# dnbaker/dashing2

Measured on AMD Instinct MI355X. Metric: all-pairs sketch comparison throughput (pairs/s), higher is better.
Workload: dtype u64

## Files before the change

### dashing2_amd/capi.py

```python
import ctypes as C
import os
import subprocess

import numpy as np

_HERE = os.path.dirname(os.path.abspath(__file__))
LIB_PATH = os.environ.get("D2G_LIB") or os.path.join(_HERE, "libd2g.so")
_lib = None

SIMILARITY, CONTAINMENT, SYMMETRIC_CONTAINMENT, POISSON_LLR, INTERSECTION, UNION_SIZE = range(6)
CMP_AUTO, CMP_DIRECT, CMP_BITSLICE, CMP_PLANES = 0, 1, 2, 3
BITSLICE_OPS_PER_GROUP_EXTRA = 1


TIME_K1, TIME_K2, TIME_K2PREP, TIME_K3, TIME_K0 = 2, 4, 8, 16, 32
TIME_KNN = 64
TIME_DEDUP = 128
TIME_FILTER = 256
TIME_KSET = 512
TIME_SCREEN = 1024


class D2GError(RuntimeError):
    def __init__(self, status, detail=""):
# ... 142 lines not shown
    "d2g_cmp_set_update_dev": (_int, [_vp, _vp, _vp, _vp]),
    "d2g_cmp_set_planes": (_int, [_vp, _vp, _vp, C.POINTER(C.c_uint), C.POINTER(_int), C.POINTER(_f32)]),
    "d2g_cmp_set_status": (_int, [_vp, _vp, _vp]),
    "d2g_cmp_set_sparse_info": (_int, [_vp, _vp, _vp, _vp]),
    "d2g_cmp_set_debug_pairs": (_int, [_vp, _vp, _vp, _vp, _sz, C.POINTER(_sz), _vp]),
    "d2g_cmp_set_sparse_detail": (_int, [_vp, _vp, _vp, _vp]),
    "d2g_sparse_bin_geometry": (_int, [_sz, C.POINTER(C.c_uint32), C.POINTER(C.c_uint32), C.POINTER(C.c_uint32), C.POINTER(_int)]),
    "d2g_warmup": (_int, [_vp, _int]),
    "d2g_device_name": (_int, [_int, C.c_char_p, _sz]),
    "d2g_comm_unique_id": (_int, [_vp]),
    "d2g_comm_create": (_int, [_vp, _vp, _int, _int, C.POINTER(_vp)]),
    "d2g_comm_create_all": (_int, [C.POINTER(_vp), _int, C.POINTER(_vp)]),
    "d2g_comm_destroy": (None, [_vp]),
    "d2g_comm_rank": (_int, [_vp]),
    "d2g_comm_world": (_int, [_vp]),
    "d2g_comm_is_rccl": (_int, [_vp]),
    "d2g_bcast_sigs": (_int, [C.POINTER(_vp), C.POINTER(_vp), _int, _vp, _sz, _sz, C.POINTER(_vp)]),
    "d2g_allpairs_create": (_int, [_vp, _vp, _sz, _sz, C.POINTER(_vp)]),
    "d2g_allpairs_destroy": (None, [_vp]),
    "d2g_allpairs_rows_held": (_int, [_vp, C.POINTER(_sz), C.POINTER(_sz)]),
    "d2g_allpairs_rows_computed": (_int, [_vp, C.POINTER(_sz), C.POINTER(_sz)]),
    "d2g_allpairs_prepare_dev": (_int, [_vp, _vp, _vp]),
    "d2g_allpairs_prepare_all": (_int, [C.POINTER(_vp), _int, C.POINTER(_vp), C.POINTER(_vp)]),
    "d2g_allpairs_operand": (_vp, [_vp]),
    "d2g_allpairs_status": (_int, [_vp, _vp]),
    "d2g_allpairs_chunks": (_int, [_vp]),
    "d2g_allpairs_set_phase_timing": (_int, [_vp, _int]),
    "d2g_allpairs_phase_times": (_int, [_vp, _int, C.POINTER(_int), _vp, _vp, _vp, _vp]),
    "d2g_allpairs_sparse_info": (_int, [_vp, _vp]),
    "d2g_allpairs_step_lut_dev": (_int, [_vp, _vp, _vp, _vp, _vp]),
    "d2g_allpairs_step_eqcount_dev": (_int, [_vp, _vp, _vp, _vp]),
    "d2g_allpairs_step_all": (_int, [C.POINTER(_vp), _int, C.POINTER(_vp), C.POINTER(_vp), C.POINTER(_vp), C.POINTER(_vp)]),
    "d2g_allpairs_enqueue_lut_dev": (_int, [_vp, _vp, _vp, _vp, _vp, _int]),
    "d2g_operand_layout": (_int, [_sz, _sz, C.POINTER(_sz), C.POINTER(_sz)]),
    "d2g_cmp_set_export_operand_dev": (_int, [_vp, _vp, _vp, _vp, _vp]),
    "d2g_cmp_set_from_planes_dev": (_int, [_vp, _sz, _sz, _vp, _vp, C.POINTER(_vp)]),
    "d2g_pack_column_slices_dev": (_int, [_vp, _vp, _sz, _sz, _int, _vp, _vp]),
    "d2g_cmp_set_destroy": (None, [_vp]),
    "d2g_cmp_set_algo": (_int, [_vp]),
    "d2g_cmp_eqcount_ut_dev": (_int, [_vp, _vp, _sz, _sz, _vp, _vp]),
    "d2g_cmp_lut_ut_dev": (_int, [_vp, _vp, _sz, _sz, _vp, _vp, _vp]),
    "d2g_cmp_ut_prefill_dev": (_int, [_vp, _vp, _sz, _sz, _vp, _vp, _vp, _vp]),
    "d2g_cmp_ut_announce_dev": (_int, [_vp, _vp, _sz, _sz, _vp, _vp, _vp]),
    "d2g_cmp_set_forget": (_int, [_vp, _vp]),
    "d2g_cmp_gtlt_ut_dev": (_int, [_vp, _vp, _sz, _sz, _vp, _vp, _vp]),
    "d2g_cmp_eqcount_rect_dev": (_int, [_vp, _vp, _sz, _sz, _sz, _sz, _vp, _vp]),
    "d2g_cmp_gtlt_rect_dev": (_int, [_vp, _vp, _sz, _sz, _sz, _sz, _vp, _vp, _vp]),
    "d2g_cmp_eqcount_ut": (_int, [_vp, _vp, _sz, _sz, _sz, _sz, _int, _vp]),
    "d2g_cmp_dist_ut": (_int, [_vp, _vp, _vp, _sz, _sz, _sz, _sz, _int, _int, _int, _int, _int, _vp]),
    "d2g_ut_partition": (_int, [_sz, _int, C.POINTER(_sz)]),
    "d2g_cmp_set_create_codes_dev": (_int, [_vp, _vp, _sz, _sz, _int, _vp, C.POINTER(_vp)]),
    "d2g_cmp_set_create_codes": (_int, [_vp, _vp, _sz, _sz, _int, C.POINTER(_vp)]),
    "d2g_cmp_set_operand_bytes": (_sz, [_vp]),
    "d2g_cmp_dist_trunc_ut": (_int, [_vp, _vp, _vp, _sz, _sz, _sz, _sz, _int, _int, _int, _int, _int, _vp]),
    "d2g_cmp_knn_dev": (_int, [_vp, _vp, _sz, _sz, _sz, C.c_uint32, _vp, _sz, _vp, _vp, _vp, _sz, _vp]),
    "d2g_knn_finish": (_int, [_vp, _vp, _vp, _sz, _sz, _vp, _sz, _int, _vp, _vp, _vp, _sz, C.POINTER(_sz), C.POINTER(_sz)]),
    "d2g_cmp_set_knn": (_int, [_vp, _vp, _sz, _sz, _vp, _int, _sz, _dbl, _sz, _sz, _vp, _vp, _vp, _sz, C.POINTER(_sz)]),
    "d2g_cmp_knn": (_int, [_vp, _vp, _sz, _sz, _sz, _sz, _int, _int, _int, _int, _sz, _dbl, _sz, _sz, _vp, _vp, _vp, _sz, C.POINTER(_sz)]),
    "d2g_cmp_dedup_dev": (_int, [_vp, _vp, C.c_uint32, _vp, _vp, _sz, _vp]),
    "d2g_dedup_clusters": (_int, [_vp, _sz, _vp, _vp, C.POINTER(_sz)]),
    "d2g_cmp_set_dedup": (_int, [_vp, _vp, _vp, _dbl, _sz, _vp]),
    "d2g_cmp_dedup": (_int, [_vp, _vp, _sz, _sz, _int, _int, _int, _int, _dbl, _sz, _vp]),
}


def sparse_info_dict(a):
    return {"sorted_operand": bool(a[0]), "tiles_listed": int(a[1]), "dense_decided_by_prepare": bool(a[2] & 1), "dense_kernel_ran": bool(a[2] & 2),
            "tiles_and_pair_list": bool(a[2] & 4), "callers_order_kept": bool(a[2] & 8), "ordering_skipped": bool(a[2] & 16), "pairs_listed": int(a[3])}


def lib():
    global _lib
    if _lib is None:
        if os.environ.get("D2G_NO_TORCH_PRELOAD") != "1":
            try:
                import torch
            except Exception:
                pass
        if not os.path.exists(LIB_PATH):
            raise OSError(f"{LIB_PATH} is missing: run `python -c 'import __graft_entry__ as g; g.build()'` "
                          "(dashing2_amd has no CPU fallback)")
        l = C.CDLL(LIB_PATH)
        for name, (res, args) in SIGNATURES.items():
            f = getattr(l, name)
            f.restype = res
            f.argtypes = args
        _lib = l
    return _lib


def _np_ptr(a):
    return a.ctypes.data if a is not None else None


class _Runs:

    def __init__(self, src, canon):
        if hasattr(src, "arrays"):
            src = tuple(src.arrays()) + (src.k,)
        elif src[0] is None:
            src = (None,) + tuple(src[1][:3]) + (src[2],)
        packed, rs, rl, go, self.k = src
        self.packed = None if packed is None else np.ascontiguousarray(packed, np.uint8)
        self.rs, self.rl, self.go = np.ascontiguousarray(rs, np.uint64), np.ascontiguousarray(rl, np.uint32), np.ascontiguousarray(go, np.uint64)
        self.n = self.go.size - 1
        self.args = (_np_ptr(self.packed), 0 if packed is None else self.packed.size, _np_ptr(self.rs), _np_ptr(self.rl), self.rs.size,
                     _np_ptr(self.go), self.n, self.k, int(canon))

    @property
    def nkmers(self):
        return int(self.rl.astype(np.int64).sum()) - (self.k - 1) * self.rl.size if self.rl.size else 0


def wang_hash(x):
    return int(lib().d2g_wang_hash(x & 0xFFFFFFFFFFFFFFFF))


def wang_hash_inverse(x):
    return int(lib().d2g_wang_hash_inverse(x & 0xFFFFFFFFFFFFFFFF))


SCREEN_MAX_KEYS = 1 << 30


def run_emissions(length, k, w=0):
    return int(lib().d2g_run_emissions(int(length), int(k), int(w)))


def screen_table_slots(ndistinct):
    s = _u64()
    rc = lib().d2g_screen_table_slots(ndistinct, C.byref(s))
    if rc:
        raise D2GError(rc)
    return int(s.value)


def epilogue_contain(matches, matchsums, S):
# ... 887 lines not shown
        return int(lib().d2g_kset_slice_bits(self._h))

    def isz_ut_dev(self, r0, r1, out_dev_ptr, stream=None):
        self.ctx._check(lib().d2g_kset_isz_ut_dev(self.ctx._h, self._h, r0, r1, out_dev_ptr, stream))

    def isz_rect_dev(self, a0, a1, b0, b1, out_dev_ptr, stream=None):
        self.ctx._check(lib().d2g_kset_isz_rect_dev(self.ctx._h, self._h, a0, a1, b0, b1, out_dev_ptr, stream))

    def close(self):
        if getattr(self, "_h", None):
            lib().d2g_kset_destroy(self._h)
            self._h = None

    __del__ = close


class OphPlan:
    def __init__(self, ctx, h, n):
        self.ctx, self._h, self.n = ctx, h, n

    def set_filter(self, filt):
        self.ctx._check(lib().d2g_oph_plan_set_filter(self._h, filt._h if filt is not None else None))
        self._filter = filt

    @property
    def nkmers(self):
        return int(lib().d2g_oph_plan_nkmers(self._h))

    @property
    def nbases(self):
        return int(lib().d2g_oph_plan_nbases(self._h))

    def close(self):
        if self._h:
            lib().d2g_oph_plan_destroy(self._h)
            self._h = None

    __del__ = close


class CmpSet:

    def __init__(self, ctx, h, N, S, owned=True):
        self.ctx, self._h, self.N, self.S, self._owned = ctx, h, N, S, owned

    @property
    def algo(self):
        return int(lib().d2g_cmp_set_algo(self._h))

    @property
    def operand_bytes(self):
        return int(lib().d2g_cmp_set_operand_bytes(self._h))

    def close(self):
        if getattr(self, "_h", None):
            if self._owned:
                lib().d2g_cmp_set_destroy(self._h)
            self._h = None

    __del__ = close

    def export_operand_dev(self, planes_out_ptr, meta_out_ptr, stream=None):
        self.ctx._check(lib().d2g_cmp_set_export_operand_dev(self.ctx._h, self._h, planes_out_ptr, meta_out_ptr, stream))

    def update_dev(self, dev_ptr, stream=None):
        self.ctx._check(lib().d2g_cmp_set_update_dev(self.ctx._h, self._h, dev_ptr, stream))

    def status(self, stream=None):
        self.ctx._check(lib().d2g_cmp_set_status(self.ctx._h, self._h, stream))

    def sparse_info(self, stream=None):
        a = np.zeros(4, np.uint32)
        self.ctx._check(lib().d2g_cmp_set_sparse_info(self.ctx._h, self._h, stream, a.ctypes.data))
        return sparse_info_dict(a)

    def sparse_detail(self, stream=None):
        a = np.zeros(10, np.uint64)
        self.ctx._check(lib().d2g_cmp_set_sparse_detail(self.ctx._h, self._h, stream, a.ctypes.data))
        return {"looked": bool(a[0]), "looked_dense": bool(a[1]), "entries": int(a[2]), "family_pairs": int(a[3]), "shared_values": int(a[4]),
                "planes": int(a[5]), "binned": bool(a[6]), "bin_cshift": int(a[7]), "schedule": "merged" if a[8] else "classic", "prepare_kernels": int(a[9])}

    def debug_pairs(self, cap=1 << 24, stream=None):
        buf = np.empty(cap, np.uint64)
        roots = np.empty(self.N, np.uint32)
        n = _sz()
        self.ctx._check(lib().d2g_cmp_set_debug_pairs(self.ctx._h, self._h, stream, buf.ctypes.data, cap, C.byref(n), roots.ctypes.data))
        e = buf[:n.value]
        e = e[e != np.uint64(0xFFFFFFFFFFFFFFFF)]
        return np.stack([(e & np.uint64(0xFFFFFFFF)).astype(np.uint32), (e >> np.uint64(32)).astype(np.uint32)], axis=1), roots

    def planes(self, stream=None):
        md, nb, mean = C.c_uint(), _int(), _f32()
        self.ctx._check(lib().d2g_cmp_set_planes(self.ctx._h, self._h, stream, C.byref(md), C.byref(nb), C.byref(mean)))
        return int(md.value), int(nb.value), float(mean.value)

    def eqcount_ut_dev(self, out_dev_ptr, r0=0, r1=None, stream=None):
        r1 = self.N if r1 is None else r1
        self.ctx._check(lib().d2g_cmp_eqcount_ut_dev(self.ctx._h, self._h, r0, r1, out_dev_ptr, stream))

    def lut_ut_dev(self, lut_dev_ptr, out_dev_ptr, r0=0, r1=None, stream=None):
        r1 = self.N if r1 is None else r1
        self.ctx._check(lib().d2g_cmp_lut_ut_dev(self.ctx._h, self._h, r0, r1, lut_dev_ptr, out_dev_ptr, stream))

    def prefill_ut_dev(self, out_dev_ptr, r0=0, r1=None, lut_dev_ptr=None, stream=None):
        r1 = self.N if r1 is None else r1
        if lut_dev_ptr is None:
# ... 252 lines not shown
```

### dashing2_amd/csrc/d2g_internal.h

```cpp
#pragma once
#include "../../include/d2g.h"
#include <hip/hip_runtime.h>
#include <cstdio>
#include <memory>
#include <string>
#include <utility>

#include <vector>
struct d2g_ctx;
int d2g_hip_status(d2g_ctx *ctx, hipError_t e, const char *what);

template <class T, bool Pinned> class d2g_owned {
    T *p_ = nullptr; size_t cap_ = 0;
public:
    d2g_owned() = default;
    d2g_owned(d2g_owned &&o) noexcept : p_(o.p_), cap_(o.cap_) { o.p_ = nullptr; o.cap_ = 0; }
    d2g_owned &operator=(d2g_owned &&o) noexcept { if (this != &o) { reset(); p_ = o.p_; cap_ = o.cap_; o.p_ = nullptr; o.cap_ = 0; } return *this; }
    ~d2g_owned() { reset(); }
    void reset() { if (p_) (void)(Pinned ? hipHostFree(p_) : hipFree(p_)); p_ = nullptr; cap_ = 0; }
    int alloc(d2g_ctx *ctx, size_t n, const char *what, unsigned flags = hipHostMallocDefault) {
        reset();
        const hipError_t e = Pinned ? hipHostMalloc((void **)&p_, n * sizeof(T), flags) : hipMalloc((void **)&p_, n * sizeof(T));
        if (e != hipSuccess) p_ = nullptr; else cap_ = n;
        return d2g_hip_status(ctx, e, what);
// ... 4 lines not shown
    T *get() const { return p_; }
    operator T *() const { return p_; }
    size_t cap() const { return cap_; }
};
template <class T> using d2g_dev = d2g_owned<T, false>;
template <class T> using d2g_pinned = d2g_owned<T, true>;

template <class H, hipError_t (*Destroy)(H)> class d2g_handle {
protected:
    H h_ = nullptr;
public:
    d2g_handle() = default;
    d2g_handle(d2g_handle &&o) noexcept : h_(o.h_) { o.h_ = nullptr; }
    d2g_handle &operator=(d2g_handle &&o) noexcept { if (this != &o) { reset(); h_ = o.h_; o.h_ = nullptr; } return *this; }
    ~d2g_handle() { reset(); }
    void reset() { if (h_) (void)Destroy(h_); h_ = nullptr; }
    operator H() const { return h_; }
};
struct d2g_stream : d2g_handle<hipStream_t, hipStreamDestroy> {
    hipError_t create(unsigned flags = hipStreamDefault) { reset(); return hipStreamCreateWithFlags(&h_, flags); }
};
struct d2g_event : d2g_handle<hipEvent_t, hipEventDestroy> {
    hipError_t create(unsigned flags = hipEventDefault) { reset(); return hipEventCreateWithFlags(&h_, flags); }
};

struct d2g_evlog {
    std::vector<d2g_event> a, b;
};

struct d2g_tuning {
    std::vector<std::pair<std::string, std::string>> kv;
    const char *get(const char *name) const {
        for (const auto &p : kv) if (p.first == name) return p.second.c_str();
        return nullptr;
    }
};
void d2g_tuning_load(d2g_tuning &t);
struct d2g_k2_tuning {
    bool sparse = true;
    size_t min_n = 8192;
    int link = 1;
    double tile_frac = 0.35;
    int olink = 1;
    int emit_big = 0;
    int ride = 63;
    int merge = 1;
    int remember = 1;
    size_t long_list = 786432;
    int predict = 1;
    int list_form = 0;
    size_t list_div = 8;
    bool sort = true;
    int tagbits_max = 31;
    int nsplit_req = 0;
};
d2g_k2_tuning d2g_k2_tuning_resolve(const d2g_tuning &t);
std::string d2g_k2_tuning_json(const d2g_ctx *ctx);
uint64_t d2g_k2_tuning_hash(const d2g_ctx *ctx);

constexpr int K3_MAXBBITS = 12;
constexpr int K3_ROUND_KEYS = 1400;
constexpr int K3_TARGET = 1024;
constexpr int K3_L1BITS = 8;
constexpr uint64_t K3_SPLIT_MIN = 4 * 1400;
struct d2g_k3_tuning {
    bool compact = false;
    bool light = true;
    uint32_t l1bits = K3_L1BITS;
    uint64_t bucket_keys = K3_TARGET;
    uint64_t sub_keys = K3_TARGET;
    uint64_t split_min = 0;
    size_t subbatch = 0;
    uint32_t round_keys = K3_ROUND_KEYS;
    double guess_scale = 1.0;
    size_t grid_per_cu = 48;
    bool gq_scale_set = false;
    double gq_scale = 2.0;
    uint64_t gq_slack = 256;
    uint64_t sort_keys = K3_TARGET;
};
struct d2g_kset_tuning {
    int split = 0;
    int pbits = -1;
};
d2g_k3_tuning d2g_k3_tuning_resolve(const d2g_tuning &t);
constexpr int MG_MAX_CHUNKS = 4;
void d2g_tuning_resolve(d2g_ctx *ctx);

struct d2g_ctx {
    int device = -1;
    d2g_tuning tune;
    d2g_k2_tuning k2;
    d2g_k3_tuning k3_tune;
    d2g_kset_tuning kset;
    int mgpu_chunks = 0;
    int num_cus = 0;
    std::string last_error;
    int timing = 0;
    d2g_evlog ev_k1, ev_k2, ev_k2prep, ev_k3, ev_k0, ev_knn;
    d2g_evlog ev_k1count;
    d2g_evlog ev_filter;
    d2g_evlog ev_k3s, ev_kset, ev_ksetprep;
    d2g_evlog ev_screen, ev_screenreduce, ev_screenbuild;
    d2g_evlog ev_dedup, ev_dedup_resolve;
    struct d2g_k3_state *k3 = nullptr;
    d2g_dev<uint32_t> knn_band;
// ... 49 lines not shown
```

### dashing2_amd/csrc/d2g_k2.h

```cpp
#pragma once
#include "d2g_internal.h"

#include <algorithm>

struct SpRider { uint32_t *out; size_t cnt; const uint32_t *vsrc; uint32_t vimm, own, piece0; };
constexpr SpRider SP_NO_RIDER{nullptr, 0, nullptr, 0u, 0xFFFFFFFFu, 0u};
constexpr int SP_FILL_PER_THREAD = 8, SP_FILL_THREADS = 256;
inline size_t sp_fill_pieces(size_t cnt) { return div_up<size_t>(cnt / 4 + 1, (size_t)SP_FILL_THREADS * SP_FILL_PER_THREAD); }
#ifndef D2G_SP_RW_M_LINK0
#define D2G_SP_RW_M_LINK0 8
#endif
#ifndef D2G_SP_RW_M_PLANES
#define D2G_SP_RW_M_PLANES 5
#endif
constexpr unsigned SP_RW_PLAN = 6, SP_RW_FLATTEN = 5, SP_RW_COUNT = 5, SP_RW_ATTACH = 5, SP_RW_SCAN = 8, SP_RW_ALL = 35;
constexpr unsigned SP_RW_M_LINK0 = D2G_SP_RW_M_LINK0, SP_RW_M_PLANES = D2G_SP_RW_M_PLANES;

struct SpInit {
    uint32_t *label = nullptr, *ones = nullptr, *zero = nullptr;
    uint32_t n = 0, owords = 0, zwords = 0;
};
#ifdef __HIPCC__
__device__ __forceinline__ void sp_init_part(const SpInit &si, size_t lin, size_t nthreads) {
    if (!si.label) return;
// ... 65 lines not shown
    size_t owner_stride = 0;
    d2g_dev<uint32_t> d_segend;
    d2g_dev<uint32_t> d_posseg;
    d2g_dev<uint32_t> d_hint;
    d2g_dev<uint32_t> d_spz;
    size_t spz_words = 0;
    uint32_t *d_lcnt = nullptr;
    uint32_t *d_gbm = nullptr;
    uint32_t *d_order = nullptr;
    uint32_t *d_plctl = nullptr;
    d2g_dev<uint32_t> d_rowpos;
    d2g_dev<uint32_t> d_rowk;
    d2g_dev<uint32_t> d_rowstream;
    d2g_dev<uint32_t> d_tiles, d_spctl; uint32_t *d_tilebm = nullptr;
    d2g_dev<uint32_t> d_tiles_full; uint32_t *d_fullctl = nullptr;
    bool full_list_valid = false;
    d2g_pinned<uint32_t> h_gaveup; uint32_t *d_gaveup = nullptr;
    d2g_stream fill_stream; d2g_event fill_fork, fill_join;
    d2g_stream samp_stream; d2g_event samp_event;
    d2g_dev<uint32_t> d_samp;
    SpDecision dec;
    SpAnnounced announced;
    SpFilled filled;
    const uint32_t *last_ctl = nullptr;
    d2g_dev<unsigned long long> d_plist;
    size_t plist_cap = 0;
    d2g_dev<unsigned long long> d_plist2;
    uint32_t *d_binc = nullptr;
    d2g_dev<uint32_t> d_bstart;
    d2g_dev<uint32_t> d_cw_ents; d2g_dev<unsigned long long> d_cw_vals; size_t cw_ecap = 0, cw_vcap = 0;
    d2g_dev<uint32_t> d_hoff;
    uint32_t nbins = 0, bin_nch = 0, bin_cshift = 10, bin_nwg = 1;
    bool bin_ok = true;
    size_t tilebm_words = 0, tiles_cap = 0;
};

struct d2g_cmp_set {
    d2g_ctx *ctx = nullptr;
    size_t N = 0, S = 0;
    size_t Npad = 0;
    int algo = D2G_CMP_DIRECT;
    d2g_dev<uint64_t> d_rows;
    d2g_dev<uint64_t> d_cols;
    d2g_dev<uint32_t> d_cplanes;
    int cplanes = 0;
    d2g_dev<uint32_t> own_planes, own_meta;
    uint32_t *d_planes = nullptr;
    d2g_dev<uint32_t> d_stream;
    size_t Nstride = 0;
    int nbits_cap = 0;
    int ntb = 0;
    uint32_t *d_meta = nullptr;
    d2g_dev<uint32_t> d_ids;
    uint32_t T = 0; int logT = 0;
    bool borrowed = false;
    bool want_exchange = false;
    d2g_dev<uint32_t> d_colcnt;
    d2g_dev<uint32_t> d_perm;
    int nsplit = 1;
    bool export_only = false;
    uint32_t *ex_planes = nullptr, *ex_meta = nullptr, *ex_status = nullptr;
    bool managed = false;
    const uint32_t *status_words = nullptr; int n_status = 0;
    std::unique_ptr<SpState> sp;
    bool sparse_ok() const { return sp != nullptr; }
    size_t ncols = 0;
    bool srt_valid = false;
    mutable bool nat_valid = false;
};
constexpr int BS_CC_STRIDE = 8;

struct PairShape;
int  finish_shape(d2g_ctx *ctx, PairShape &sh, unsigned rb);

int  d2g_planes_gtlt(d2g_ctx *ctx, const d2g_cmp_set *set, const PairShape &sh, uint32_t *gt, uint32_t *lt, hipStream_t s);
int  d2g_planes_eq(d2g_ctx *ctx, const d2g_cmp_set *set, const PairShape &sh, uint32_t *eq, hipStream_t s);

void d2g_bitslice_geometry(d2g_cmp_set *set);
int  d2g_bitslice_alloc(d2g_ctx *ctx, d2g_cmp_set *set);
int  d2g_bitslice_prepare(d2g_ctx *ctx, d2g_cmp_set *set, hipStream_t s);
int  d2g_bitslice_export(d2g_ctx *ctx, d2g_cmp_set *set, hipStream_t s);
int  d2g_bitslice_alloc_stream(d2g_ctx *ctx, d2g_cmp_set *set);
int  d2g_bitslice_ensure_natural(d2g_ctx *ctx, const d2g_cmp_set *set, hipStream_t s);
int  d2g_bitslice_managed_sparse_alloc(d2g_ctx *ctx, d2g_cmp_set *set);
int  d2g_bitslice_managed_ready(d2g_ctx *ctx, d2g_cmp_set *set, hipStream_t s);
int  d2g_bitslice_sparse_info(d2g_ctx *ctx, const d2g_cmp_set *set, hipStream_t s, uint32_t *out4);
int  d2g_bitslice_sparse_detail(d2g_ctx *ctx, const d2g_cmp_set *set, hipStream_t s, uint64_t *out10);
SpInit d2g_bitslice_sp_init(const d2g_cmp_set *set);
int  d2g_bitslice_debug_read(d2g_ctx *ctx, const d2g_cmp_set *set, hipStream_t s, uint64_t *pairs_out, size_t cap, size_t *npairs, uint32_t *root_out);
int  d2g_bitslice_status(d2g_ctx *ctx, const d2g_cmp_set *set, hipStream_t s);
int  d2g_bitslice_exporter_create(d2g_ctx *ctx, size_t N, size_t S_local, d2g_cmp_set **out);
void d2g_bitslice_set_export_target(d2g_cmp_set *set, uint32_t *planes, uint32_t *meta, uint32_t *status);
int  d2g_bitslice_prepare_slice(d2g_ctx *ctx, d2g_cmp_set *set, const uint64_t *rows_dev, hipStream_t s);
int  d2g_bitslice_derive_groups(d2g_ctx *ctx, const d2g_cmp_set *set, int g0, int g1, hipStream_t s);
int  d2g_bitslice_ut(d2g_ctx *ctx, const d2g_cmp_set *set, size_t r0, size_t r1, uint32_t *eq_out,
                     const float *lut, float *fout, hipStream_t s);
int  d2g_bitslice_prefill(d2g_ctx *ctx, d2g_cmp_set *set, size_t r0, size_t r1, uint32_t *eq_out, const float *lut, float *fout, hipStream_t s);
int  d2g_bitslice_announce(d2g_ctx *ctx, d2g_cmp_set *set, size_t r0, size_t r1, uint32_t *eq_out, const float *lut, float *fout);
void d2g_bitslice_forget(d2g_cmp_set *set);
int  d2g_bitslice_rect(d2g_ctx *ctx, const d2g_cmp_set *set, size_t a0, size_t a1, size_t b0, size_t b1,
                       uint32_t *eq_out, hipStream_t s);
```

### dashing2_amd/csrc/d2g_k2.hip

```cpp
#include "d2g_internal.h"
#include "d2g_k2.h"
#include "d2g_k2_shape.h"
#include <algorithm>
#include <new>
#include <vector>

namespace {

constexpr int K2_THREADS = 256;
constexpr int K2_IW = 8;
constexpr int K2_JR = 4;
constexpr int K2_RB = 4 * K2_IW;
constexpr int K2_CB = 64 * K2_JR;
constexpr int K2_TC = 2;

}
int finish_shape(d2g_ctx *ctx, PairShape &sh, unsigned rb) {
    sh.rb = rb;
    sh.nrt = (unsigned)div_up<size_t>(sh.i_hi - sh.i_lo, rb);
    sh.ct0 = (unsigned)(sh.j_lo / 256);
    sh.nct = (unsigned)(div_up<size_t>(sh.j_hi, 256) - sh.ct0);
    size_t total = 0;
    for (unsigned c = 0; c < sh.nct; ++c) total += tiles_in_column(sh, c);
    D2G_CHECK(ctx, total < (1ull << 31), "pair tile grid too large; shard rows");
// ... 98 lines not shown
    } else {
        uint32_t val[K2_IW][K2_JR];
#pragma unroll
        for (int i = 0; i < K2_IW; ++i)
#pragma unroll
            for (int c = 0; c < K2_JR; ++c) val[i][c] = store.value(acc[i][c]);
#pragma unroll
        for (int i = 0; i < K2_IW; ++i) {
            const size_t ii = iw0 + i;
            if (ii >= sh.i_hi) break;
#pragma unroll
            for (int c = 0; c < K2_JR; ++c) {
                const size_t jj = j0 + lane + 64 * c;
                if (jj < sh.j_hi && jj >= sh.j_lo && (!sh.ut || jj > ii)) store.put(out_pos(sh, ii, jj), val[i][c]);
            }
        }
    }
}

template <bool GTLT, class Store>
int launch_direct(d2g_ctx *ctx, const d2g_cmp_set *set, PairShape sh, Store store, hipStream_t s) {
    if (int rc = finish_shape(ctx, sh, K2_RB)) return rc;
    if (sh.nvalid_total == 0) return D2G_OK;
    d2g_timer tm(ctx, &ctx->ev_k2, s);
    hipLaunchKernelGGL((k2_direct_kernel<GTLT, Store>), dim3(sh.per_xcd * 8), dim3(K2_THREADS), 0, s,
                       set->d_rows, set->d_cols, set->S, set->Npad, sh, store);
    tm.stop();
    D2G_HIP(ctx, hipGetLastError());
    return D2G_OK;
}

}

namespace {
__global__ __launch_bounds__(256) void k2_pack_slices_kernel(const uint64_t *__restrict__ rows, size_t n, size_t S, size_t Sl,
                                                             uint64_t *__restrict__ out) {
    const size_t i = (size_t)blockIdx.x * 256 + threadIdx.x;
    if (i >= n * S) return;
    const size_t r = i / S, c = i - r * S, q = c / Sl;
    out[(q * n + r) * Sl + (c - q * Sl)] = rows[i];
}
}


extern "C" {

void d2g_cmp_set_destroy(d2g_cmp_set *set) {
    if (!set) return;
    (void)hipSetDevice(set->ctx->device);
    delete set;
}

int d2g_cmp_set_algo(const d2g_cmp_set *set) { return set ? set->algo : D2G_ERR_INVALID; }

size_t d2g_cmp_set_operand_bytes(const d2g_cmp_set *set) {
    if (!set) return 0;
    return (set->d_rows.cap() + set->d_cols.cap()) * sizeof(uint64_t) +
           (set->own_planes.cap() + set->d_stream.cap() + (set->sp ? set->sp->d_stream_s.cap() : 0) + set->d_cplanes.cap()) * sizeof(uint32_t);
}

#define D2G_NO_CODE_SET(ctx, set, what) D2G_CHECK(ctx, (set)->algo != D2G_CMP_PLANES, what ": not available for a set of truncated codes")

static int cmp_set_load(d2g_ctx *ctx, d2g_cmp_set *set, const uint64_t *sig_bits_dev, hipStream_t s) {
    const size_t N = set->N, S = set->S;
    if (set->d_rows) D2G_HIP(ctx, hipMemcpyAsync(set->d_rows, sig_bits_dev, N * S * sizeof(uint64_t), hipMemcpyDeviceToDevice, s));
    d2g_timer tm(ctx, &ctx->ev_k2prep, s);
    launch_transpose(ctx, sig_bits_dev, set->d_cols, N, S, set->Npad, set->algo == D2G_CMP_BITSLICE ? set->d_meta + set->ntb : nullptr,
                     set->algo == D2G_CMP_BITSLICE ? d2g_bitslice_sp_init(set) : SpInit{}, s);
    int rc = D2G_OK;
    if (set->algo == D2G_CMP_BITSLICE) rc = d2g_bitslice_prepare(ctx, set, s);
    tm.stop();
    if (rc) return rc;
    D2G_HIP(ctx, hipGetLastError());
    return D2G_OK;
}

}

int d2g_bitslice_prepare_slice(d2g_ctx *ctx, d2g_cmp_set *set, const uint64_t *rows_dev, hipStream_t s) {
    d2g_timer tm(ctx, &ctx->ev_k2prep, s);
    launch_transpose(ctx, rows_dev, set->d_cols, set->N, set->S, set->Npad, set->d_meta + set->ntb, d2g_bitslice_sp_init(set), s);
    const int rc = d2g_bitslice_prepare(ctx, set, s);
    tm.stop();
    if (rc) return rc;
    D2G_HIP(ctx, hipGetLastError());
    return D2G_OK;
}

extern "C" {

int d2g_cmp_set_create_dev(d2g_ctx *ctx, const uint64_t *sig_bits_dev, size_t N, size_t S, int algo,
                           void *stream, d2g_cmp_set **out) {
    if (!ctx || !out) return D2G_ERR_INVALID;
    *out = nullptr;
    D2G_CHECK(ctx, N >= 1 && S >= 1, "cmp_set: empty matrix");
    D2G_CHECK(ctx, S < (1ull << 31), "cmp_set: sketchsize too large");
    D2G_CHECK(ctx, sig_bits_dev != nullptr, "cmp_set: null signatures");
    D2G_CHECK(ctx, algo == D2G_CMP_AUTO || algo == D2G_CMP_DIRECT || algo == D2G_CMP_BITSLICE, "cmp_set: bad algo");
    D2G_HIP(ctx, hipSetDevice(ctx->device));
    hipStream_t s = as_stream(stream);
    d2g_cmp_set *set = new (std::nothrow) d2g_cmp_set();
    if (!set) return D2G_ERR_NOMEM;
    set->ctx = ctx; set->N = N; set->S = S;
    set->Npad = div_up<size_t>(N, K2_CB) * K2_CB;
    if (int rc = set->d_cols.alloc(ctx, set->Npad * S, "cmp_set alloc")) { d2g_cmp_set_destroy(set); return rc; }
    set->algo = D2G_CMP_DIRECT;
// ... 326 lines not shown
```

### dashing2_amd/csrc/d2g_k2_bitslice.hip

```cpp
#include "d2g_internal.h"
#include "d2g_k2.h"
#include "d2g_k2_shape.h"
#include <chrono>
#include <cstring>
#include <algorithm>
#include <vector>

namespace {

typedef uint32_t u32x16 __attribute__((ext_vector_type(16)));
typedef u32x16 __attribute__((aligned(4))) u32x16_u;
constexpr uint32_t BS_EMPTY = 0xFFFFFFFFu;
constexpr int BS_RANK_THREADS = 1024;

constexpr uint32_t BS_DUP = 0x80000000u;
constexpr uint32_t BS_UNIQ = 0x80000000u;
constexpr uint32_t BS_PENDING = 0x40000000u;
constexpr int BS_LOG_TLDS_MAX = 15;

__device__ __forceinline__ uint32_t bs_hash(uint64_t v, int logT) {
    return (uint32_t)((v * 0x9E3779B97F4A7C15ull) >> (64 - logT));
}

constexpr uint32_t BS_SPLIT_SHIFT = 28, BS_RANK_MASK = (1u << BS_SPLIT_SHIFT) - 1u;
#ifdef D2G_RANK_TRACE
__device__ unsigned long long g_rank_trace[8192 * 16];
#define RK_STAMP(k) do { if (threadIdx.x == 0 && blockIdx.x < 8192 && (k) < 16) g_rank_trace[blockIdx.x * 16 + (k)] = __builtin_amdgcn_s_memrealtime(); } while (0)
#else
#define RK_STAMP(k) do { } while (0)
#endif
template <bool MULTI, bool FAST>
__global__ __launch_bounds__(BS_RANK_THREADS) void bs_rank_kernel(const uint64_t *__restrict__ cols, size_t N, size_t Npad,
                                                                  uint32_t T, int logT, uint32_t *ids_all, uint32_t *colcnt,
                                                                  uint32_t *status, int tagbits_max, uint32_t S, int nsplit,
                                                                  uint32_t *__restrict__ owner_all, size_t ostride) {
    extern __shared__ __attribute__((aligned(16))) uint32_t own[];
    const uint32_t split = MULTI ? blockIdx.x / S : 0u;
    const size_t t = MULTI ? blockIdx.x - split * S : blockIdx.x;
    const uint32_t htag = (MULTI && nsplit > 1) ? split << BS_SPLIT_SHIFT : 0u;
    const uint64_t *col = cols + t * Npad;
    uint32_t *ids = ids_all + t * Npad;
    const int tid = threadIdx.x;
    const int logTl = logT < BS_LOG_TLDS_MAX ? logT : BS_LOG_TLDS_MAX;
    const uint32_t Tl = 1u << logTl, mask = Tl - 1, nparts = MULTI ? (T >> logTl) : 1u;
    const uint32_t part_lo = MULTI ? split * (nparts / (uint32_t)nsplit) : 0u, part_hi = MULTI ? part_lo + nparts / (uint32_t)nsplit : 1u;
    __shared__ uint32_t wave_tot[BS_RANK_THREADS / 64];
    __shared__ uint32_t running;
    constexpr uint32_t BS_MAXFIX = 64;
    __shared__ uint32_t nfix, fix_j[BS_MAXFIX], fix_h[BS_MAXFIX];
    RK_STAMP(0);
    if (tid == 0) { running = 1; nfix = 0; }
    const int lane = tid & 63, wave = tid >> 6;
    uint32_t *owner = (owner_all && nsplit == 1) ? owner_all + t * ostride : nullptr;
    const int ib0 = 32 - __clz((uint32_t)N);
    const uint32_t ownmask = (ib0 >= 32 ? 0xFFFFFFFFu : (1u << ib0) - 1u) & ~BS_DUP;

    auto compact = [&]() {
        uint32_t cnt = 0;
        for (uint32_t h = tid; h < Tl; h += BS_RANK_THREADS) {
            const uint32_t cur = own[h];
            cnt += (cur != BS_EMPTY) && (cur & BS_DUP);
        }
        uint32_t incl = cnt;
        for (int o = 1; o < 64; o <<= 1) { const uint32_t x = __shfl_up(incl, o); if (lane >= o) incl += x; }
        if (lane == 63) wave_tot[wave] = incl;
        __syncthreads();
        uint32_t woff = 0, tot = 0;
        for (int w = 0; w < BS_RANK_THREADS / 64; ++w) {
            const uint32_t x = wave_tot[w];
            if (w < wave) woff += x;
            tot += x;
        }
        uint32_t r = running + woff + (incl - cnt);
        for (uint32_t h = tid; h < Tl; h += BS_RANK_THREADS) {
            const uint32_t cur = own[h];
            if (cur != BS_EMPTY) {
                if ((cur & BS_DUP) && owner) owner[r - 1] = cur & ownmask;
                own[h] = (cur & BS_DUP) ? (r++ | htag) : BS_UNIQ;
            }
        }
        __syncthreads();
        if (tid == 0) running += tot;
        __syncthreads();
    };
    const int ib = 32 - __clz((uint32_t)N);
    const uint32_t idxmask = (ib >= 32 ? 0xFFFFFFFFu : (1u << ib) - 1u) & ~BS_DUP;
    const uint32_t tagfield = ~BS_DUP & ~idxmask & (ib + tagbits_max >= 31 ? 0xFFFFFFFFu : (1u << (ib + tagbits_max)) - 1u);
    auto slot_word = [&](uint64_t prod, uint32_t j) {
        return j | ((uint32_t)((prod << logT) >> 33) & tagfield);
    };
    auto insert = [&](uint64_t v, uint32_t j, uint32_t h) {
        const uint32_t mine = slot_word(v * 0x9E3779B97F4A7C15ull, j);
        for (uint32_t probes = 0; probes < Tl; ++probes) {
            const uint32_t cur = atomicCAS(&own[h], BS_EMPTY, mine);
            if (cur == BS_EMPTY) return h;
            if (!((cur ^ mine) & tagfield) && col[cur & idxmask] == v) {
                if (!(cur & BS_DUP)) atomicOr(&own[h], BS_DUP);
                return h;
            }
            h = (h + 1) & mask;
        }
        atomicOr(status, 1u);
        return h;
    };

    constexpr int PF = 12;
    if constexpr (FAST) {
        uint64_t v[PF];
        uint32_t hs[PF];
#pragma unroll
        for (int i = 0; i < PF; ++i) {
            const size_t j = (size_t)i * BS_RANK_THREADS + tid;
            v[i] = j < N ? col[j] : 0;
        }
        for (uint32_t h = tid; h < Tl; h += BS_RANK_THREADS) own[h] = BS_EMPTY;
        __syncthreads();
        RK_STAMP(1);
        uint32_t candidate = 0;
#pragma unroll
        for (int i = 0; i < PF; ++i) {
            const size_t j = (size_t)i * BS_RANK_THREADS + tid;
            hs[i] = 0;
            if (j < N) {
                const uint64_t prod = v[i] * 0x9E3779B97F4A7C15ull;
                const uint32_t mine = slot_word(prod, (uint32_t)j);
                uint32_t h = (uint32_t)(prod >> (64 - logT)) & mask, probes = 0;
                for (; probes < Tl; ++probes) {
                    const uint32_t cur = atomicCAS(&own[h], BS_EMPTY, mine);
                    if (cur == BS_EMPTY) break;
                    if (!((cur ^ mine) & tagfield)) { candidate |= 1u << i; break; }
                    h = (h + 1) & mask;
                }
                if (probes == Tl) atomicOr(status, 1u);
                hs[i] = h;
            }
        }
        constexpr int CB = 2;
        uint32_t redo = 0;
#ifdef D2G_RANK_TRACE
        __syncthreads();
        RK_STAMP(2);
#endif
#pragma unroll
        for (int c = 0; c < PF; c += CB) {
            uint32_t o[CB];
            uint64_t w[CB];
#pragma unroll
            for (int g = 0; g < CB; ++g)
                if (candidate >> (c + g) & 1) o[g] = own[hs[c + g]];
#pragma unroll
            for (int g = 0; g < CB; ++g)
                if (candidate >> (c + g) & 1) w[g] = col[o[g] & idxmask];
#pragma unroll
            for (int g = 0; g < CB; ++g)
                if (candidate >> (c + g) & 1) {
                    if (w[g] == v[c + g]) {
                        if (!(o[g] & BS_DUP)) atomicOr(&own[hs[c + g]], BS_DUP);
                    } else redo |= 1u << (c + g);
                }
            __builtin_amdgcn_sched_barrier(0);
        }
        const uint32_t skip = redo;
        while (redo) {
            const int i = __ffs(redo) - 1;
            redo &= redo - 1;
            const uint32_t j = (uint32_t)i * BS_RANK_THREADS + tid;
            const uint64_t vv = col[j];
            const uint32_t h2 = insert(vv, j, bs_hash(vv, logT) & mask);
            const uint32_t k = atomicAdd(&nfix, 1u);
            if (k < BS_MAXFIX) { fix_j[k] = j; fix_h[k] = h2; }
            else atomicOr(status, 1u);
        }
        __syncthreads();
        RK_STAMP(3);
        compact();
        RK_STAMP(4);
#pragma unroll
        for (int i = 0; i < PF; ++i) {
            const size_t j = (size_t)i * BS_RANK_THREADS + tid;
            if (j < N && !(skip >> i & 1)) ids[j] = own[hs[i]];
        }
#ifdef D2G_RANK_TRACE
        __syncthreads();
        RK_STAMP(5);
#endif
        for (uint32_t k = tid; k < nfix && k < BS_MAXFIX; k += BS_RANK_THREADS) ids[fix_j[k]] = own[fix_h[k]];
        if (tid == 0) { colcnt[t * BS_CC_STRIDE] = running - 1; colcnt[t * BS_CC_STRIDE + 5] = running - 1; }
        return;
    }

    const bool tagged = MULTI && nsplit > 1;
    for (uint32_t part = part_lo; part < part_hi; ++part) {
        const uint32_t ptag = BS_PENDING | (tagged ? part << 15 : 0u);
        for (uint32_t h = tid; h < Tl; h += BS_RANK_THREADS) own[h] = BS_EMPTY;
        __syncthreads();
        constexpr int PG = 8;
        const bool mine_known = N <= (size_t)8 * PG * BS_RANK_THREADS;
        unsigned long long mine_all = 0;
        int batch = 0;
        for (size_t j0 = 0; j0 < N; j0 += (size_t)PG * BS_RANK_THREADS) {
            uint64_t v[PG];
            uint32_t hs[PG];
#pragma unroll
            for (int i = 0; i < PG; ++i) {
                const size_t j = j0 + (size_t)i * BS_RANK_THREADS + tid;
                v[i] = j < N ? col[j] : 0;
            }
            uint32_t mineb = 0, candidate = 0, redo = 0;
#pragma unroll
            for (int i = 0; i < PG; ++i) {
                const size_t j = j0 + (size_t)i * BS_RANK_THREADS + tid;
                const uint64_t prod = v[i] * 0x9E3779B97F4A7C15ull;
                const uint32_t hh = (uint32_t)(prod >> (64 - logT));
                hs[i] = 0;
                if (j < N && (!MULTI || (hh >> logTl) == part)) {
                    mineb |= 1u << i;
                    const uint32_t mine = slot_word(prod, (uint32_t)j);
                    uint32_t h = hh & mask, probes = 0;
                    for (; probes < Tl; ++probes) {
                        const uint32_t cur = atomicCAS(&own[h], BS_EMPTY, mine);
                        if (cur == BS_EMPTY) break;
                        if (!((cur ^ mine) & tagfield)) { candidate |= 1u << i; break; }
                        h = (h + 1) & mask;
                    }
                    if (probes == Tl) atomicOr(status, 1u);
                    hs[i] = h;
                }
            }
            {
                uint32_t o[PG];
                uint64_t w[PG];
#pragma unroll
                for (int i = 0; i < PG; ++i)
                    if (candidate >> i & 1) o[i] = own[hs[i]];
#pragma unroll
                for (int i = 0; i < PG; ++i)
                    if (candidate >> i & 1) w[i] = col[o[i] & idxmask];
#pragma unroll
                for (int i = 0; i < PG; ++i)
                    if (candidate >> i & 1) {
                        if (w[i] == v[i]) { if (!(o[i] & BS_DUP)) atomicOr(&own[hs[i]], BS_DUP); }
                        else redo |= 1u << i;
                    }
            }
#pragma unroll
            for (int i = 0; i < PG; ++i) {
                const size_t j = j0 + (size_t)i * BS_RANK_THREADS + tid;
                if ((mineb & ~redo) >> i & 1) ids[j] = hs[i] | (MULTI ? ptag : 0u);
                else if (MULTI && !tagged && part == 0 && j < N && !(redo >> i & 1)) ids[j] = 0;
            }
            while (redo) {
                const int i = __ffs(redo) - 1;
                redo &= redo - 1;
                const size_t j = j0 + (size_t)i * BS_RANK_THREADS + tid;
                const uint64_t vv = col[j];
                ids[j] = insert(vv, (uint32_t)j, bs_hash(vv, logT) & mask) | (MULTI ? ptag : 0u);
            }
            if (batch < 8) mine_all |= (unsigned long long)mineb << (8 * batch);
            ++batch;
        }
        __syncthreads();
        RK_STAMP(1 + 2 * (part - part_lo));
        compact();
        batch = 0;
        for (size_t j0 = 0; j0 < N; j0 += (size_t)PG * BS_RANK_THREADS, ++batch) {
            uint32_t sl[PG];
            const uint32_t mb = mine_known ? (uint32_t)(mine_all >> (8 * batch)) & 0xFFu : 0xFFu;
#pragma unroll
            for (int i = 0; i < PG; ++i) {
                const size_t j = j0 + (size_t)i * BS_RANK_THREADS + tid;
                sl[i] = (j < N && (mb >> i & 1)) ? ids[j] : 0;
            }
#pragma unroll
            for (int i = 0; i < PG; ++i) {
                const size_t j = j0 + (size_t)i * BS_RANK_THREADS + tid;
                if (j < N && (mb >> i & 1) && (mine_known || !MULTI || (tagged ? (sl[i] & ~0x7FFFu) == ptag : (sl[i] & BS_PENDING) != 0)))
                    ids[j] = own[sl[i] & (tagged ? 0x7FFFu : ~BS_PENDING)];
            }
        }
        __syncthreads();
        RK_STAMP(2 + 2 * (part - part_lo));
    }
    if (tid == 0) { colcnt[t * BS_CC_STRIDE + split] = running - 1; if (nsplit == 1) colcnt[t * BS_CC_STRIDE + 5] = running - 1; }
}

__device__ __forceinline__ int live_planes(const uint32_t *meta, int tb) {
    const uint32_t md = meta[tb];
    return md <= 1 ? 1 : 32 - __clz(md);
}

__device__ __forceinline__ size_t stream_slot(const uint32_t *meta, int tb) {
    size_t q = 0;
    for (int t = 0; t < tb; ++t) q += (size_t)live_planes(meta, t);
    return q;
}

__device__ __forceinline__ size_t stream_slot_wave(const uint32_t *meta, int tb) {
    const int lane = threadIdx.x & 63;
    uint32_t q = 0;
    for (int t0 = 0; t0 < tb; t0 += 64) {
        const int t = t0 + lane;
        uint32_t v = t < tb ? (uint32_t)live_planes(meta, t) : 0u;
        for (int o = 32; o > 0; o >>= 1) v += __shfl_xor(v, o);
        q += v;
    }
    return (size_t)__builtin_amdgcn_readfirstlane(q);
}

__device__ __forceinline__ void sp_ride_piece(const SpRider &r, size_t piece) {
    typedef uint32_t u32x4 __attribute__((ext_vector_type(4)));
    const uint32_t v = r.vsrc ? r.vsrc[0] : r.vimm;
    const size_t head = min(r.cnt, (size_t)((16 - ((uintptr_t)r.out & 15)) & 15) / 4);
    u32x4 *body = reinterpret_cast<u32x4 *>(r.out + head);
    const size_t nb = (r.cnt - head) / 4;
    const size_t end = min((piece + 1) * (size_t)2048, nb);
    for (size_t i = piece * 2048 + threadIdx.x; i < end; i += blockDim.x) __builtin_nontemporal_store(u32x4{v, v, v, v}, &body[i]);
    if (piece == 0) {
        if (threadIdx.x < head) r.out[threadIdx.x] = v;
        const size_t tail0 = head + nb * 4;
        if (tail0 + threadIdx.x < r.cnt) r.out[tail0 + threadIdx.x] = v;
    }
}
__device__ __forceinline__ void sp_ride(const SpRider &r) { sp_ride_piece(r, (size_t)r.piece0 + (blockIdx.x - r.own)); }
#define SP_RIDE_OR_WORK(r) do { if (blockIdx.x >= (r).own) { sp_ride(r); return; } } while (0)
__global__ __launch_bounds__(256) void sp_side_fill_kernel(SpRider r, uint32_t pieces) {
    for (size_t p = blockIdx.x; p < pieces; p += gridDim.x) sp_ride_piece(r, p);
}
constexpr uint32_t SP_SIDE_FILL_PIECES = 32768;
inline unsigned sp_side_fill_grid(const d2g_ctx *ctx, uint32_t pieces, size_t words, size_t N, size_t S) {
    const double need = (double)words * 4.0 / (1.3 * 21.0 * (double)N * ((double)S / 1024.0));
// ... 65 lines not shown
            if (t < Spad) d2s[t] = d2;
            unsigned long long todo = __ballot(t < Spad);
            while (todo) {
                const int k = __shfl(cls, __ffsll((long long)todo) - 1);
                const unsigned long long m = __ballot(cls == k && t < Spad);
                const uint32_t ci = (uint32_t)(31 - k) * nchunk + t / 64;
                if (cls == k && t < Spad) mine[it] = ci << 6 | (uint32_t)__popcll(m & ((1ull << lane) - 1));
                if (lane == 0) cell[(uint32_t)(31 - k) * nchunk + (t - lane) / 64] = __popcll(m);
                todo &= ~m;
            }
        }
    }
    __syncthreads();
    {
        constexpr int CPT = 32 * (BS_PLAN_MAXS / 64) / T;
        const uint32_t c0 = (uint32_t)CPT * tid;
        uint32_t v[CPT], sum = 0;
#pragma unroll
        for (int x = 0; x < CPT; ++x) { v[x] = c0 + x < ncell ? cell[c0 + x] : 0u; sum += v[x]; }
        uint32_t incl = sum;
        for (int o = 1; o < 64; o <<= 1) { const uint32_t x = __shfl_up(incl, o); if (lane >= o) incl += x; }
        if (lane == 63) wave_tot[wave] = incl;
        __syncthreads();
        uint32_t ex = incl - sum;
        for (int w = 0; w < wave; ++w) ex += wave_tot[w];
#pragma unroll
        for (int x = 0; x < CPT; ++x) { if (c0 + x < ncell) cell[c0 + x] = ex; ex += v[x]; }
    }
    __syncthreads();
#pragma unroll
    for (int it = 0; it < IT; ++it) {
        const uint32_t t = (uint32_t)it * T + tid;
        if (t < Spad) perm_s[cell[mine[it] >> 6] + (mine[it] & 63u)] = (uint16_t)t;
    }
    __syncthreads();
    for (uint32_t p = tid; p < Spad; p += T) { const uint32_t t = perm_s[p]; perm[p] = t < S ? t : BS_NOCOL; }
    for (int g = tid; g < ntb; g += T) {
        uint32_t mx = 0;
        for (uint32_t x = 0; x < 32; ++x) mx = max(mx, d2s[perm_s[(uint32_t)g * 32 + x]]);
        meta[g] = mx + 1;
        if (ex_meta) ex_meta[g] = mx + 1;
    }
}

__global__ __launch_bounds__(BS_PLAN_THREADS) void bs_colplan_kernel(BsPlanArgs pa, SpRider rider) {
    SP_RIDE_OR_WORK(rider);
    extern __shared__ __attribute__((aligned(16))) uint32_t plan_lds[];
    bs_colplan_body<BS_PLAN_THREADS>(pa, bs_plan_lds(plan_lds, (uint32_t)pa.ntb * 32u));
}

constexpr int BS_FORM_STREAM = 1, BS_FORM_EXCHANGE = 2;
constexpr size_t BS_SLACK = 64;
struct BsPlanesArgs {
    const uint32_t *ids; size_t N, Npad; uint32_t *planes, *stream; size_t Nstride; int nbits_cap; const uint32_t *meta; int forms;
    const uint32_t *perm, *colcnt, *sperm;
};
BsPlanesArgs planes_args_of(const d2g_cmp_set *set, uint32_t *planes, int forms) {
    return BsPlanesArgs{set->d_ids, set->N, set->Npad, planes, set->d_stream, set->Nstride, set->nbits_cap, set->d_meta, forms, set->d_perm, set->d_colcnt, nullptr};
}
template <bool SPLIT>
__device__ __forceinline__ void bs_planes_body(const BsPlanesArgs &a, size_t bx, size_t tb) {
    const uint32_t *__restrict__ ids = a.ids, *__restrict__ meta = a.meta, *__restrict__ perm = a.perm, *__restrict__ colcnt = a.colcnt, *__restrict__ sperm = a.sperm;
    uint32_t *__restrict__ planes = a.planes, *__restrict__ stream = a.stream;
    const size_t N = a.N, Npad = a.Npad, Nstride = a.Nstride;
    const int nbits_cap = a.nbits_cap, forms = a.forms;
    const size_t jpos = bx * 256 + threadIdx.x;
    const size_t slot = (forms & BS_FORM_STREAM) ? stream_slot_wave(meta, (int)tb) : 0;
    if (jpos >= Nstride) return;
    const size_t j = sperm ? (size_t)sperm[jpos] : jpos;
    const int nbits = live_planes(meta, (int)tb);
    typedef const u32x16_u __attribute__((address_space(4))) *slots_ptr;
    const u32x16_u pa = *(slots_ptr)(uintptr_t)(perm + tb * 32), pb = *(slots_ptr)(uintptr_t)(perm + tb * 32 + 16);
    uint32_t id[32];
#pragma unroll
    for (int x = 0; x < 32; ++x) {
        const uint32_t t = x < 16 ? pa[x] : pb[x - 16];
        const bool real = t != BS_NOCOL && j < N;
        uint32_t w = real ? ids[(size_t)t * Npad + j] : 0u;
        if (SPLIT && real && !(w >> 31)) w = (w & BS_RANK_MASK) + colcnt[(size_t)t * BS_CC_STRIDE + (w >> BS_SPLIT_SHIFT)];
        id[x] = w;
    }
    uint32_t u = 0;
#pragma unroll
    for (int x = 0; x < 32; ++x) u |= (id[x] >> 31) << x;
    uint32_t *dst = planes + tb * (size_t)(nbits_cap + 1) * Nstride + jpos;
    const bool ex = forms & BS_FORM_EXCHANGE, st = forms & BS_FORM_STREAM;
    uint32_t *sdst = st ? stream + slot * 2 * Nstride + jpos : nullptr;
    for (int b = 0; b < nbits; ++b) {
        uint32_t w = 0;
#pragma unroll
        for (int x = 0; x < 32; ++x) w |= ((id[x] >> b) & 1u) << x;
        if (ex) dst[(size_t)b * Nstride] = w;
        if (st) {
            sdst[(size_t)(2 * b) * Nstride] = w;
            sdst[(size_t)(2 * b + 1) * Nstride] = w | u;
        }
    }
    if (ex) {
        uint32_t uw = u;
        if (jpos >= Npad && jpos < Npad + 32) { const uint32_t t = perm[tb * 32 + (jpos - Npad)]; uw = t != BS_NOCOL ? colcnt[(size_t)t * BS_CC_STRIDE + 4] : 0u; }
        dst[(size_t)nbits_cap * Nstride] = uw;
    }
}
template <bool SPLIT>
__global__ __launch_bounds__(256) void bs_planes_kernel(BsPlanesArgs a) { bs_planes_body<SPLIT>(a, blockIdx.x, blockIdx.y); }

__global__ __launch_bounds__(256) void bs_derive_kernel(const uint32_t *__restrict__ planes, uint32_t *__restrict__ stream,
                                                        size_t Nstride, int nbits_cap, const uint32_t *__restrict__ meta, int tb0) {
    const size_t j = (size_t)blockIdx.x * 256 + threadIdx.x;
    const size_t tb = (size_t)tb0 + blockIdx.y;
    if (j >= Nstride) return;
    const int nbits = live_planes(meta, (int)tb);
    const uint32_t *src = planes + tb * (size_t)(nbits_cap + 1) * Nstride + j;
    uint32_t *sdst = stream + stream_slot(meta, (int)tb) * 2 * Nstride + j;
    const uint32_t u = j + BS_SLACK < Nstride ? src[(size_t)nbits_cap * Nstride] : 0u;
    for (int b = 0; b < nbits; ++b) {
        const uint32_t w = src[(size_t)b * Nstride];
        sdst[(size_t)(2 * b) * Nstride] = w;
        sdst[(size_t)(2 * b + 1) * Nstride] = w | u;
    }
}

constexpr int BS_THREADS = 256;
constexpr int BS_CB = 256;

constexpr unsigned BITOP3_C_OR_A_XOR_B = 0xAA | (0xF0 ^ 0xCC);

#ifndef D2G_BS_WPE
#define D2G_BS_WPE 7
#endif
#ifndef D2G_BS_JR
#define D2G_BS_JR 2
#endif
constexpr int BS_IW = 16;
constexpr int BS_JR = D2G_BS_JR;

__device__ __forceinline__ bool sp_dense_mode(const uint32_t *__restrict__ ctl, uint32_t cand);
#include "d2g_k2_patch.h"


template <int JR>
struct BsOperands {
    u32x16_u sa;
    uint32_t vb[JR];
};

template <int JR>
__device__ __forceinline__ BsOperands<JR> bs_fetch(const uint32_t *&ptr, uint32_t coff, size_t step) {
    __builtin_amdgcn_s_waitcnt(0xc07f);
    __builtin_amdgcn_sched_barrier(0);
    BsOperands<JR> o;
    typedef const u32x16_u __attribute__((address_space(4))) *row_words_ptr;
    o.sa = *(row_words_ptr)(uintptr_t)ptr;
    uint32_t co = coff;
    asm volatile("" : "+v"(co));
#pragma unroll
    for (int c = 0; c < JR; ++c)
        o.vb[c] = *reinterpret_cast<const uint32_t *>(reinterpret_cast<const char *>(ptr) + co + 256 * c);
// ... 114 lines not shown

#include "d2g_k2_sparse.h"

int refresh_borrowed(d2g_ctx *ctx, const d2g_cmp_set *set, hipStream_t s) {
    if (!set->borrowed || set->managed) return D2G_OK;
    return d2g_bitslice_derive_groups(ctx, set, 0, set->ntb, s);
}


template <class Store>
int launch_bitslice(d2g_ctx *ctx, const d2g_cmp_set *set, PairShape sh, Store store, hipStream_t s) {
    if (int rc = finish_shape(ctx, sh, BS_JR == 2 ? 32u : 64u)) return rc;
    if (sh.nvalid_total == 0) return D2G_OK;
    if (int rc = refresh_borrowed(ctx, set, s)) return rc;
    if (int rc = d2g_bitslice_ensure_natural(ctx, set, s)) return rc;
    d2g_timer tm(ctx, &ctx->ev_k2, s);
    hipLaunchKernelGGL((k2_bitslice_kernel<BS_JR, Store>), dim3(sh.per_xcd * 8), dim3(BS_THREADS), 0, s, set->d_stream,
                       set->Nstride, set->d_meta, set->ntb, (uint32_t)set->S, sh, store, (const uint32_t *)nullptr, 0u, SpPatchArgs{});
    tm.stop();
    D2G_HIP(ctx, hipGetLastError());
    return D2G_OK;
}

}

void d2g_bitslice_geometry(d2g_cmp_set *set) {
    set->nbits_cap = 1;
    while ((1ull << set->nbits_cap) < set->N / 2 + 2) ++set->nbits_cap;
    set->ntb = (int)div_up<size_t>(set->S, 32);
    set->Nstride = set->Npad + BS_SLACK;
}

int d2g_bitslice_alloc_stream(d2g_ctx *ctx, d2g_cmp_set *set) {
    return set->d_stream.alloc(ctx, ((size_t)set->ntb * set->nbits_cap + 1) * 2 * set->Nstride, "bitslice alloc");
}

namespace {
int alloc_prepare_workspace(d2g_ctx *ctx, d2g_cmp_set *set) {
    const size_t N = set->N, S = set->S, Npad = set->Npad;
    if (N >= (1ull << 30)) { ctx->last_error = "bitslice: N too large"; return D2G_ERR_UNSUPPORTED; }
    d2g_bitslice_geometry(set);
    set->T = 64; set->logT = 6;
    while ((uint64_t)set->T * 2 < (uint64_t)N * 3) { set->T <<= 1; ++set->logT; }
    set->nsplit = 1;
    if (set->logT > BS_LOG_TLDS_MAX && N < (1ull << BS_SPLIT_SHIFT)) {
        const uint32_t nparts = set->T >> BS_LOG_TLDS_MAX;
        int want = 1;
        while (want < 4 && (uint32_t)want * 2 <= nparts && S * (size_t)want < (size_t)std::max(ctx->num_cus, 1)) want *= 2;
        if (ctx->k2.nsplit_req && (uint32_t)ctx->k2.nsplit_req <= nparts) want = ctx->k2.nsplit_req;
        set->nsplit = want;
    }
    const char *what = "bitslice alloc";
    int rc;
    if ((rc = set->d_ids.alloc(ctx, S * Npad, what)) ||
        (rc = d2g_hip_status(ctx, hipMemset(set->d_ids, 0, S * Npad * sizeof(uint32_t)), what)) ||
        (rc = set->d_colcnt.alloc(ctx, S * BS_CC_STRIDE, what)) ||
        (rc = set->d_perm.alloc(ctx, (size_t)set->ntb * 32, what)) ||
        (rc = set->own_meta.alloc(ctx, (size_t)(set->ntb + 4), what)) ||
        (rc = d2g_hip_status(ctx, hipMemset(set->own_meta, 0, (size_t)(set->ntb + 4) * sizeof(uint32_t)), what))) return rc;
    set->d_meta = set->own_meta;
    return D2G_OK;
}
int launch_planes(d2g_ctx *ctx, const d2g_cmp_set *set, uint32_t *planes, int forms, hipStream_t s) {
    const dim3 grid((unsigned)div_up<size_t>(set->Nstride, 256), (unsigned)set->ntb);
    const bool split = set->logT > BS_LOG_TLDS_MAX && set->nsplit > 1;
    hipLaunchKernelGGL(split ? bs_planes_kernel<true> : bs_planes_kernel<false>, grid, dim3(256), 0, s, planes_args_of(set, planes, forms));
    D2G_HIP(ctx, hipGetLastError());
    return D2G_OK;
}
struct JoinOnExit {
    hipStream_t s; hipEvent_t ev = nullptr;
    ~JoinOnExit() { if (ev) (void)hipStreamWaitEvent(s, ev, 0); }
};
}

int d2g_bitslice_alloc(d2g_ctx *ctx, d2g_cmp_set *set) {
    if (int rc = alloc_prepare_workspace(ctx, set)) return rc;
    if (int rc = set->own_planes.alloc(ctx, (size_t)set->ntb * (set->nbits_cap + 1) * set->Nstride, "bitslice alloc")) return rc;
    set->d_planes = set->own_planes;
    if (int rc = d2g_bitslice_alloc_stream(ctx, set)) return rc;
    set->ncols = set->S;
    if (sparse_enabled(ctx, set->N) && set->S < 65536 && sp_alloc(ctx, set) != D2G_OK) (void)hipGetLastError();
    if (set->sparse_ok() && set->nsplit == 1) {
        set->sp->owner_stride = set->N / 2 + 8;
        if (set->sp->d_owner.alloc(ctx, set->S * set->sp->owner_stride, "bitslice owner alloc") != D2G_OK) (void)hipGetLastError();
    }
    return D2G_OK;
}

int d2g_bitslice_prepare(d2g_ctx *ctx, d2g_cmp_set *set, hipStream_t s) {
    const size_t N = set->N, S = set->S, Npad = set->Npad;
    SpState *const sp = set->sp.get();
    const bool sparse_path = sp && !set->export_only && !set->want_exchange;
    JoinOnExit join{s};
    if (sp) {
        sp->dec.skip_cached = sparse_path ? (sp_will_skip(ctx, *sp) ? 1 : 0) : -1;
        sp->announced.begin(ctx->k2.ride, sparse_path && sp->dec.skip_cached != 1);
    }
    if (sp && sp->announced.riding() >= SP_SIDE_FILL_PIECES) {
        if (!sp->fill_stream) {
            if (sp->fill_stream.create(hipStreamNonBlocking) != hipSuccess || sp->fill_fork.create(hipEventDisableTiming) != hipSuccess ||
                sp->fill_join.create(hipEventDisableTiming) != hipSuccess) { (void)hipGetLastError(); sp->fill_stream.reset(); sp->fill_fork.reset(); sp->fill_join.reset(); }
        }
        if (sp->fill_stream) {
            hipStream_t fs = sp->fill_stream;
            D2G_HIP(ctx, hipEventRecord(sp->fill_fork, s));
            D2G_HIP(ctx, hipStreamWaitEvent(fs, sp->fill_fork, 0));
            join.ev = sp->fill_join;
            const uint32_t pieces = sp->announced.riding();
            const SpRider all = sp->announced.take_all();
            const unsigned fgrid = sp_side_fill_grid(ctx, pieces, all.cnt, N, S);
            hipLaunchKernelGGL(sp_side_fill_kernel, dim3(fgrid), dim3(256), 0, fs, all, pieces);
            D2G_HIP(ctx, hipEventRecord(sp->fill_join, fs));
        }
    }
    const bool multi = set->logT > BS_LOG_TLDS_MAX;
    const int nsplit = multi ? set->nsplit : 1;
    {
        const int logTl = set->logT < BS_LOG_TLDS_MAX ? set->logT : BS_LOG_TLDS_MAX;
        const size_t lds = (size_t(1) << logTl) * sizeof(uint32_t);
        void (*kern)(const uint64_t *, size_t, size_t, uint32_t, int, uint32_t *, uint32_t *, uint32_t *, int, uint32_t, int, uint32_t *, size_t) = bs_rank_kernel<false, false>;
        if (multi) kern = bs_rank_kernel<true, false>;
        else if (N <= (size_t)12 * BS_RANK_THREADS) kern = bs_rank_kernel<false, true>;
        if (lds > 48 * 1024)
            D2G_HIP(ctx, hipFuncSetAttribute((const void *)kern, hipFuncAttributeMaxDynamicSharedMemorySize, (int)lds));
        if (nsplit > 1) D2G_HIP(ctx, hipMemsetAsync(set->d_ids, 0, S * Npad * sizeof(uint32_t), s));
        hipLaunchKernelGGL(kern, dim3((unsigned)(S * nsplit)), dim3(BS_RANK_THREADS), lds, s, set->d_cols, N, Npad, set->T, set->logT,
                           set->d_ids, set->d_colcnt, set->d_meta + set->ntb, ctx->k2.tagbits_max, (uint32_t)S, nsplit,
                           (sp && nsplit == 1) ? sp->d_owner.get() : (uint32_t *)nullptr, sp ? sp->owner_stride : 0);
        if (sp) sp->dec.kernels = 2 + (join.ev ? 1 : 0);
        const bool look = sparse_path && sp_sample_due(ctx, set);
        if (look) { if (int rc = sp_sample_enqueue(ctx, set, s)) return rc; if (sp->dec.sample_pending) sp->dec.kernels += 2; }
        const bool merged = sparse_path && !look && ctx->k2.merge && nsplit == 1 && sp->d_owner && ctx->k2.olink && ctx->k2.link && sp->dec.skip_cached != 1;
        if (sp) sp->dec.merged = merged;
        if (!merged) {
            unsigned g = 1; const SpRider rd = sp ? sp->announced.take(1, SP_RW_PLAN, false, 1, &g) : SP_NO_RIDER;
            const BsPlanArgs pa{set->d_colcnt, (uint32_t)S, set->ntb, nsplit, set->d_perm, set->d_meta, set->d_meta + set->ntb, set->ex_meta, set->ex_status, ctx->k2.sort ? 1 : 0};
            hipLaunchKernelGGL(bs_colplan_kernel, dim3(g), dim3(BS_PLAN_THREADS), bs_plan_lds_words((uint32_t)set->ntb * 32u, pa.sort) * 4, s, pa, rd);
            if (sp) sp->dec.kernels += 1;
        }
    }
    if (sparse_path) {
        if (!sp->dec.merged) { if (int rc = launch_planes(ctx, set, set->d_planes, BS_FORM_STREAM, s)) return rc; sp->dec.kernels += 1; }
        if (int rc = sp_sample_collect(ctx, set, s)) return rc;
        if (int rc = sp_prepare_order(ctx, set, nsplit > 1, s)) return rc;
        if (int rc = sp_permute(ctx, set, s)) return rc;
        set->srt_valid = true; set->nat_valid = true;
        if (sp->announced.riding()) sp->filled.set_by_riders(sp->announced);
        else sp->filled.void_after_prepare();
        sp->announced.served();
        D2G_HIP(ctx, hipGetLastError());
        return D2G_OK;
    }
    if (sp) sp->announced.served();
    const int forms = set->export_only ? BS_FORM_EXCHANGE : (BS_FORM_STREAM | (set->want_exchange ? BS_FORM_EXCHANGE : 0));
    if (int rc = launch_planes(ctx, set, set->export_only ? set->ex_planes : set->d_planes, forms, s)) return rc;
    if (sp) sp->dec.kernels += 1;
    set->srt_valid = false; set->nat_valid = true;
    return D2G_OK;
}

SpInit d2g_bitslice_sp_init(const d2g_cmp_set *set) { return sp_init_of(set); }

int d2g_bitslice_ensure_natural(d2g_ctx *ctx, const d2g_cmp_set *set, hipStream_t s) {
    if (set->nat_valid || set->borrowed || set->export_only) return D2G_OK;
    if (int rc = launch_planes(ctx, set, set->d_planes, BS_FORM_STREAM, s)) return rc;
    set->nat_valid = true;
    return D2G_OK;
}

int d2g_bitslice_export(d2g_ctx *ctx, d2g_cmp_set *set, hipStream_t s) {
    if (set->borrowed || set->want_exchange || set->export_only) return D2G_OK;
    set->want_exchange = true;
    return launch_planes(ctx, set, set->d_planes, BS_FORM_EXCHANGE, s);
}

int d2g_bitslice_exporter_create(d2g_ctx *ctx, size_t N, size_t S_local, d2g_cmp_set **out) {
    *out = nullptr;
    d2g_cmp_set *set = new (std::nothrow) d2g_cmp_set();
    if (!set) return D2G_ERR_NOMEM;
    set->ctx = ctx; set->N = N; set->S = S_local;
// ... 120 lines not shown
    return D2G_OK;
}

int d2g_bitslice_sparse_detail(d2g_ctx *ctx, const d2g_cmp_set *set, hipStream_t s, uint64_t *out8) {
    uint32_t binned = 0;
    if (set->sp) D2G_HIP(ctx, hipMemcpyAsync(&binned, set->sp->d_plctl + SP_PL_BINNED, 4, hipMemcpyDeviceToHost, s));
    D2G_HIP(ctx, hipStreamSynchronize(s));
    if (!set->sp) return D2G_OK;
    const SpState &sp = *set->sp;
    out8[0] = sp.dec.looked ? 1 : 0; out8[1] = sp.dec.looked_dense ? 1 : 0;
    if (sp.dec.looked) for (int x = 0; x < 4; ++x) out8[2 + x] = sp.dec.samp_sums[x];
    out8[6] = binned ? 1 : 0; out8[7] = sp.bin_cshift;
    out8[8] = sp.dec.merged ? 1 : 0; out8[9] = sp.dec.kernels;
    return D2G_OK;
}

int d2g_sparse_bin_geometry(size_t N, uint32_t *cshift, uint32_t *nch, uint32_t *nbins, int *binned_ok) {
    if (!N) return D2G_ERR_INVALID;
    const SpBinGeom g = sp_bin_geometry(N);
    if (cshift) *cshift = g.cshift;
    if (nch) *nch = g.nch;
    if (nbins) *nbins = g.nbins;
    if (binned_ok) *binned_ok = g.ok ? 1 : 0;
    return D2G_OK;
}

int d2g_bitslice_debug_read(d2g_ctx *ctx, const d2g_cmp_set *set, hipStream_t s, uint64_t *pairs_out, size_t cap, size_t *npairs, uint32_t *root_out ) {
    *npairs = 0;
    if (!set->srt_valid || !set->sp) { D2G_HIP(ctx, hipStreamSynchronize(s)); return D2G_OK; }
    const SpState &sp = *set->sp;
    uint32_t n = 0;
    D2G_HIP(ctx, hipMemcpyAsync(&n, sp.d_plctl, 4, hipMemcpyDeviceToHost, s));
    D2G_HIP(ctx, hipStreamSynchronize(s));
    const size_t m = std::min<size_t>(std::min<size_t>(n, sp.plist_cap), cap);
    if (m && pairs_out) D2G_HIP(ctx, hipMemcpy(pairs_out, sp.d_plist, m * 8, hipMemcpyDeviceToHost));
    if (root_out) D2G_HIP(ctx, hipMemcpy(root_out, sp.d_label + set->Npad, set->N * 4, hipMemcpyDeviceToHost));
    *npairs = m;
    return D2G_OK;
}

uint64_t d2g_k2_tuning_hash(const d2g_ctx *ctx) {
    const d2g_k2_tuning &t = ctx->k2;
    const long long v[] = {t.sparse, (long long)t.min_n, t.link, (long long)(t.tile_frac * 1e6), t.olink, t.emit_big, t.ride, t.remember, (long long)t.list_div, (long long)t.long_list,
                           t.list_form, t.predict, t.sort ? 1 : 0, t.tagbits_max, t.nsplit_req, t.merge};
    uint64_t h = 1469598103934665603ull;
    for (long long x : v) for (int b = 0; b < 8; ++b) { h ^= (uint64_t)(x >> (8 * b)) & 0xFF; h *= 1099511628211ull; }
    return h;
}

std::string d2g_k2_tuning_json(const d2g_ctx *ctx) {
    const d2g_k2_tuning &t = ctx->k2;
    char b[640];
    std::snprintf(b, sizeof b, "{\"D2G_BS_SPARSE\": %d, \"D2G_BS_SPARSE_MIN_N\": %zu, \"D2G_BS_SORT\": %d, \"D2G_SP_LINK\": %d, \"D2G_SP_OLINK\": %d, \"D2G_SP_TILE_FRAC\": %.3f, "
                  "\"D2G_SP_LIST_DIV\": %zu, \"D2G_SP_LONG_LIST\": %zu, \"D2G_SP_LIST_FORM\": %d, \"D2G_SP_PREDICT\": %d, \"D2G_SP_REMEMBER\": %d, \"D2G_SP_RIDE\": %d, \"D2G_SP_EMIT_BIG\": %d, \"D2G_K2_MERGE\": %d}",
                  t.sparse ? 1 : 0, t.min_n, t.sort ? 1 : 0, t.link, t.olink, t.tile_frac, t.list_div, t.long_list, t.list_form, t.predict, t.remember, t.ride, t.emit_big, t.merge);
    return b;
}

void d2g_warm_k2_bitslice() { hipFuncAttributes a; (void)hipFuncGetAttributes(&a, reinterpret_cast<const void *>(&bs_colplan_kernel)); }

#ifdef D2G_RANK_TRACE
extern "C" int d2g_debug_rank_trace(unsigned long long *out, size_t n) {
    return hipMemcpyFromSymbol(out, HIP_SYMBOL(g_rank_trace), std::min<size_t>(n, 8192 * 16) * 8) == hipSuccess ? 0 : -1;
}
#endif
#ifdef D2G_SP_TRACE
extern "C" int d2g_debug_emit_trace(unsigned long long *out, size_t n) {
    return hipMemcpyFromSymbol(out, HIP_SYMBOL(g_emit_trace), std::min<size_t>(n, 4096 * 16) * 8) == hipSuccess ? 0 : -1;
}
extern "C" int d2g_debug_sp_trace(unsigned long long *out, size_t n) {
    return hipMemcpyFromSymbol(out, HIP_SYMBOL(g_sp_trace), std::min<size_t>(n, 16384 * 8) * 8) == hipSuccess ? 0 : -1;
}
#endif
```

### dashing2_amd/csrc/d2g_k2_sparse.h

```cpp
constexpr uint32_t SP_NONE = 0xFFFFFFFFu;
constexpr uint32_t SP_SAMPLE_ROWS = 16, SP_SAMPLE_FAM = 4, SP_SAMPLE_COLS = 32;
constexpr unsigned long long SP_NULL_ENTRY = ~0ull;
#ifndef D2G_SP_KS
#define D2G_SP_KS 8
#endif
#ifndef D2G_SP_WPE
#define D2G_SP_WPE 8
#endif

__device__ __forceinline__ uint32_t sp_rank(uint32_t w, const uint32_t *__restrict__ colcnt, size_t t, bool split) {
    if ((w >> 31) || w == 0) return 0;
    return split ? (w & BS_RANK_MASK) + colcnt[t * BS_CC_STRIDE + (w >> BS_SPLIT_SHIFT)] : w;
}

__device__ __forceinline__ uint32_t sp_ld(const uint32_t *p) { return __hip_atomic_load(p, __ATOMIC_RELAXED, __HIP_MEMORY_SCOPE_AGENT); }

__device__ __forceinline__ uint32_t sp_find(uint32_t *label, uint32_t l) {
    for (int h = 0; h < 64; ++h) {
        const uint32_t p = sp_ld(&label[l]);
        if (p == l) break;
        const uint32_t g = sp_ld(&label[p]);
        if (g != p) label[l] = g;
        l = p;
    }
    return l;
}
__device__ __forceinline__ bool sp_union(uint32_t *label, uint32_t a, uint32_t b) {
    for (int it = 0; it < 64; ++it) {
        a = sp_find(label, a); b = sp_find(label, b);
        if (a == b) return true;
        if (a < b) { const uint32_t x = a; a = b; b = x; }
        if (atomicCAS(&label[a], a, b) == a) return true;
    }
    return false;
}

constexpr uint32_t SP_UDONE = 0x40000000u, SP_R2MASK = 0x3FFFFFFFu;
template <int MODE>
__global__ __launch_bounds__(1024) void sp_link_kernel(const uint32_t *__restrict__ ids, size_t N, size_t Npad, uint32_t ncols, const uint32_t *__restrict__ colcnt,
                                                       int split, uint32_t cap, uint32_t stride, uint32_t *label, uint32_t *__restrict__ hint) {
    extern __shared__ uint32_t sp_l[];
    const size_t pair = (size_t)blockIdx.x * stride;
    const size_t t1 = 2 * pair, t2 = t1 + 1;
    if (t2 >= ncols) return;
    const uint32_t d2 = colcnt[t1 * BS_CC_STRIDE + 4];
    if (d2 == 0) return;
    const uint32_t nv = min(d2, cap), T = blockDim.x;
    uint32_t *r2 = sp_l, *mn = sp_l + nv, *any = sp_l + 2 * (size_t)nv;
    for (uint32_t r = threadIdx.x; r < (MODE ? 2u : 3u) * nv; r += T) sp_l[r] = SP_NONE;
    __syncthreads();
    constexpr int U = 4;
    for (size_t j0 = 0; j0 < N; j0 += (size_t)T * U) {
        uint32_t w1[U], w2[U], lb[U];
#pragma unroll
        for (int x = 0; x < U; ++x) {
            const size_t j = j0 + (size_t)x * T + threadIdx.x;
            w1[x] = j < N ? ids[t1 * Npad + j] : 0u;
            w2[x] = j < N ? ids[t2 * Npad + j] : 0u;
            lb[x] = j < N ? sp_ld(&label[j]) : SP_NONE;
        }
#pragma unroll
        for (int x = 0; x < U; ++x) {
            const uint32_t j = (uint32_t)(j0 + (size_t)x * T + threadIdx.x);
            const uint32_t a = sp_rank(w1[x], colcnt, t1, split != 0), b = sp_rank(w2[x], colcnt, t2, split != 0);
            if (!a || a > nv) continue;
            if (MODE == 0) any[a - 1] = j;
            if (!b) continue;
            const uint32_t old = atomicCAS(&r2[a - 1], SP_NONE, b);
            if (old == SP_NONE || (old & SP_R2MASK) == b) {
                atomicMin(&mn[a - 1], lb[x]);
            }
        }
    }
    __syncthreads();
    uint32_t *myhint = hint + (size_t)(pair & 1u) * Npad;
    for (size_t j0 = 0; j0 < N; j0 += (size_t)T * U) {
        uint32_t w1[U], w2[U], lb[U];
#pragma unroll
        for (int x = 0; x < U; ++x) {
            const size_t j = j0 + (size_t)x * T + threadIdx.x;
            w1[x] = j < N ? ids[t1 * Npad + j] : 0u;
            w2[x] = j < N ? ids[t2 * Npad + j] : 0u;
            lb[x] = j < N ? sp_ld(&label[j]) : 0u;
        }
#pragma unroll
        for (int x = 0; x < U; ++x) {
            const uint32_t j = (uint32_t)(j0 + (size_t)x * T + threadIdx.x);
            const uint32_t a = sp_rank(w1[x], colcnt, t1, split != 0), b = sp_rank(w2[x], colcnt, t2, split != 0);
            if (!a || a > nv) continue;
            const uint32_t rr = r2[a - 1];
            const bool match = b && rr != SP_NONE && (rr & SP_R2MASK) == b;
            if (MODE == 0) {
                if (match) {
                    const uint32_t m = mn[a - 1];
                    if (m < lb[x]) label[j] = m;
                } else {
                    const uint32_t h = any[a - 1];
                    if (h != j) myhint[j] = h;
                }
            } else if (match) {
                const uint32_t m = mn[a - 1];
                if (m != lb[x] && !(atomicOr(&r2[a - 1], SP_UDONE) & SP_UDONE)) (void)sp_union(label, lb[x], m);
            }
        }
    }
}

constexpr uint32_t SP_OWNER_MASK = 0x7FFFFFFFu;
struct SpOlinkArgs { const uint32_t *ids; size_t N, Npad; uint32_t ncols; uint32_t *owner; size_t ostride; uint32_t stride; uint32_t *label, *hint; };
template <int MODE>
__device__ __forceinline__ void sp_olink_body(const SpOlinkArgs &a, size_t bx, size_t by) {
    const uint32_t *__restrict__ ids = a.ids;
    uint32_t *__restrict__ owner = a.owner, *label = a.label, *__restrict__ hint = a.hint;
    const size_t N = a.N, Npad = a.Npad, ostride = a.ostride;
    const size_t pair = by * a.stride;
    const size_t t1 = 2 * pair, t2 = t1 + 1;
    if (t2 >= a.ncols) return;
    const size_t j0 = (bx * 256 + threadIdx.x) * 4;
    if (j0 >= N) return;
    typedef uint32_t u32x4 __attribute__((ext_vector_type(4)));
    const u32x4 w1 = *reinterpret_cast<const u32x4 *>(ids + t1 * Npad + j0);
    const u32x4 w2 = *reinterpret_cast<const u32x4 *>(ids + t2 * Npad + j0);
    const u32x4 lb = *reinterpret_cast<const u32x4 *>(label + j0);
    uint32_t *myhint = hint + (size_t)(pair & 1u) * Npad;
    uint32_t o[4], r2o[4], lo[4];
#pragma unroll
    for (int x = 0; x < 4; ++x) {
        const uint32_t r1 = w1[x];
        o[x] = (r1 && !(r1 >> 31) && j0 + x < N) ? owner[t1 * ostride + r1 - 1] & SP_OWNER_MASK : SP_NONE;
    }
#pragma unroll
    for (int x = 0; x < 4; ++x) {
        const bool live = o[x] != SP_NONE && o[x] != (uint32_t)(j0 + x);
        r2o[x] = live ? ids[t2 * Npad + o[x]] : 0u;
        lo[x] = live ? label[o[x]] : 0u;
        if (!live) o[x] = SP_NONE;
    }
#pragma unroll
    for (int x = 0; x < 4; ++x) {
        if (o[x] == SP_NONE) continue;
        const uint32_t j = (uint32_t)(j0 + x), r2 = w2[x];
        const bool match = r2 && !(r2 >> 31) && r2 == r2o[x];
        if (MODE == 0) {
            if (match) {
                if (lo[x] < lb[x]) label[j] = lo[x]; else if (lb[x] < lo[x]) label[o[x]] = lb[x];
            } else myhint[j] = o[x];
        } else if (match && lb[x] != lo[x]) {
            uint32_t *ow = &owner[t1 * ostride + w1[x] - 1];
            if (!(atomicOr(ow, ~SP_OWNER_MASK) & ~SP_OWNER_MASK)) (void)sp_union(label, lb[x], lo[x]);
        }
    }
}
template <int MODE>
__global__ __launch_bounds__(256) void sp_olink_kernel(SpOlinkArgs a) { sp_olink_body<MODE>(a, blockIdx.x, blockIdx.y); }

__device__ __forceinline__ void sp_flatten_body(uint32_t *label, size_t N, size_t bx) {
    const size_t j = bx * 256 + threadIdx.x;
    if (j >= N) return;
    uint32_t l = (uint32_t)j;
    for (int h = 0; h < 64; ++h) {
        const uint32_t p = label[l];
        if (p == l) break;
        const uint32_t g = label[p];
        if (g != p) label[l] = g;
        l = p;
    }
    if (label[l] == l) label[j] = l;
}
__global__ __launch_bounds__(256) void sp_flatten_kernel(uint32_t *label, size_t N, SpRider rider) {
    SP_RIDE_OR_WORK(rider);
    sp_flatten_body(label, N, blockIdx.x);
}

__global__ __launch_bounds__(256) void sp_link0_plan_kernel(BsPlanArgs pa, SpOlinkArgs la, uint32_t nx, SpRider rider) {
    SP_RIDE_OR_WORK(rider);
    extern __shared__ __attribute__((aligned(16))) uint32_t plan_lds[];
    if (blockIdx.x == 0) { bs_colplan_body<256>(pa, bs_plan_lds(plan_lds, (uint32_t)pa.ntb * 32u)); return; }
    const uint32_t b = blockIdx.x - 1u;
    sp_olink_body<0>(la, b % nx, b / nx);
}
__global__ __launch_bounds__(256) void bs_planes_flatten_kernel(BsPlanesArgs a, uint32_t gx, uint32_t nflat, uint32_t *label, SpRider rider) {
    SP_RIDE_OR_WORK(rider);
    if (blockIdx.x < nflat) { sp_flatten_body(label, a.N, blockIdx.x); return; }
    const uint32_t b = blockIdx.x - nflat;
    bs_planes_body<false>(a, b % gx, b / gx);
}

__global__ __launch_bounds__(256) void sp_attach_kernel(uint32_t *__restrict__ root, uint32_t *__restrict__ cnt, const uint32_t *__restrict__ hint, size_t N, size_t Npad,
                                                        const uint32_t *__restrict__ order, SpRider rider) {
    SP_RIDE_OR_WORK(rider);
    const size_t j = (size_t)blockIdx.x * 256 + threadIdx.x;
    if (j >= N || order[2]) return;
    if (root[j] != (uint32_t)j || sp_ld(&cnt[j]) != 1u) return;
    const uint32_t a = hint[j], b = hint[Npad + j];
    if (a == SP_NONE && b == SP_NONE) return;
    const uint32_t ra = a != SP_NONE ? sp_ld(&root[a]) : SP_NONE, rb = b != SP_NONE ? sp_ld(&root[b]) : SP_NONE;
    if (ra != SP_NONE && rb != SP_NONE && ra != rb) return;
    const uint32_t r = ra != SP_NONE ? ra : rb;
    if (r == (uint32_t)j || sp_ld(&cnt[r]) < 2u) return;
    root[j] = r;
    atomicAdd(&cnt[r], 1u);
    cnt[j] = 0;
}

template <int NW = 16>
__device__ __forceinline__ uint32_t sp_block_scan(uint32_t v, uint32_t *wave_tot, uint32_t *total) {
    const int lane = threadIdx.x & 63, wave = threadIdx.x >> 6;
    uint32_t incl = v;
    for (int o = 1; o < 64; o <<= 1) { const uint32_t x = __shfl_up(incl, o); if (lane >= o) incl += x; }
    __syncthreads();
    if (lane == 63) wave_tot[wave] = incl;
    __syncthreads();
    uint32_t woff = 0, tot = 0;
    for (int w = 0; w < NW; ++w) { const uint32_t x = wave_tot[w]; if (w < wave) woff += x; tot += x; }
    *total = tot;
    return woff + incl - v;
}

template <int NW>
__device__ __forceinline__ unsigned long long sp_block_scan64(unsigned long long v, unsigned long long *wave_tot, unsigned long long *total) {
    const int lane = threadIdx.x & 63, wave = threadIdx.x >> 6;
    unsigned long long incl = v;
    for (int o = 1; o < 64; o <<= 1) { const unsigned long long x = __shfl_up(incl, o); if (lane >= o) incl += x; }
    __syncthreads();
    if (lane == 63) wave_tot[wave] = incl;
    __syncthreads();
    unsigned long long woff = 0, tot = 0;
    for (int w = 0; w < NW; ++w) { const unsigned long long x = wave_tot[w]; if (w < wave) woff += x; tot += x; }
    *total = tot;
    return woff + incl - v;
}

__device__ __forceinline__ uint32_t sp_seg_est(uint32_t c) {
    c = min(c, 32768u);
    return c >= 32 ? 16u * ((c + 31) / 32 + 1) * ((c + 255) / 256 + 1) : (c >= 2 ? c : 0u);
}

constexpr int SP_MAX_HOPS = 64;
// ... 79 lines not shown
    __syncthreads();
    if (tid == 0) { const uint32_t keep = (s_big || order[2] || s_est > seg_tile_limit + 1024) ? 1u : 0u; order[0] = keep; *gaveup = keep; }
}
__device__ __forceinline__ void sp_segtiles(uint32_t a, uint32_t b, uint32_t CW, uint32_t *__restrict__ gbm) {
    if (b - a < 2) return;
    const uint32_t cb0 = a >> 8, cb1 = (b - 1) >> 8;
    for (uint32_t rb = a >> 5; rb <= (b - 1) >> 5; ++rb)
        for (uint32_t cw = cb0 >> 5; cw <= cb1 >> 5; ++cw) {
            const uint32_t lo = cw == (cb0 >> 5) ? (cb0 & 31) : 0u, hi = cw == (cb1 >> 5) ? (cb1 & 31) : 31u;
            const uint32_t m = (hi == 31 ? 0xFFFFFFFFu : ((1u << (hi + 1)) - 1u)) & ~((1u << lo) - 1u);
            atomicOr(&gbm[(size_t)rb * CW + cw], m);
        }
}
__global__ __launch_bounds__(256) void sp_place_kernel(const uint32_t *__restrict__ root, size_t N, size_t Nstride, uint32_t *__restrict__ cnt,
                                                        uint32_t *__restrict__ sperm, uint32_t *__restrict__ sinv, const uint32_t *__restrict__ order,
                                                        const uint32_t *__restrict__ seg_start, const uint32_t *__restrict__ seg_end, uint32_t CW, uint32_t *__restrict__ gbm,
                                                        uint2 *__restrict__ posseg, SpRider rider) {
    SP_RIDE_OR_WORK(rider);
    const size_t j = (size_t)blockIdx.x * 256 + threadIdx.x;
    const bool live = j < N;
    if (!live && j < Nstride) sperm[j] = SP_NONE;
    if (order[0]) { if (live) { sperm[j] = (uint32_t)j; sinv[j] = (uint32_t)j; } return; }
    const uint32_t r = live ? root[j] : SP_NONE;
    if (live && r == (uint32_t)j) sp_segtiles(seg_start[j], seg_end[j], CW, gbm);
    const int lane = threadIdx.x & 63;
    uint32_t p = 0;
    const unsigned long long alive = __ballot(live);
    if (!alive) return;
    const uint32_t lead = __shfl(r, __ffsll((long long)alive) - 1);
    const unsigned long long m = __ballot(live && r == lead);
    const int first = __ffsll((long long)m) - 1;
    uint32_t base = 0;
    if (lane == first) base = atomicAdd(&cnt[lead], (uint32_t)__popcll(m));
    base = __shfl(base, first);
    if (live && r == lead) p = base + (uint32_t)__popcll(m & ((1ull << lane) - 1));
    else if (live) p = atomicAdd(&cnt[r], 1u);
    if (live) { sperm[p] = (uint32_t)j; sinv[j] = p; posseg[p] = uint2{seg_start[r], seg_end[r]}; }
}

struct SpColWork { uint32_t *ents; uint4 *vals; uint32_t ecap, vcap; };
__device__ __forceinline__ unsigned long long *sp_pl_streams(uint32_t *plctl) { return reinterpret_cast<unsigned long long *>(plctl + 8 + (((uintptr_t)(plctl + 8) >> 2) & 1u)); }
__device__ __forceinline__ unsigned long long *sp_pl_proj(uint32_t *plctl) { return reinterpret_cast<unsigned long long *>(plctl + 1 + (((uintptr_t)(plctl + 1) >> 2) & 1u)); }

#ifndef D2G_SP_EMIT_T
#define D2G_SP_EMIT_T 512
#endif
#ifdef D2G_SP_TRACE
__device__ unsigned long long g_emit_trace[4096 * 16];
#define EM_STAMP(k) do { if (threadIdx.x == 0 && blockIdx.x < 4096 && lo == 0) g_emit_trace[blockIdx.x * 16 + (k)] = __builtin_amdgcn_s_memrealtime(); } while (0)
#else
#define EM_STAMP(k) do { } while (0)
#endif
constexpr uint32_t SP_EMIT_VCAP = 1536, SP_EMIT_ECAP = 32768, SP_EMIT_T = D2G_SP_EMIT_T;
__global__ __launch_bounds__(SP_EMIT_T) __attribute__((amdgpu_waves_per_eu(8, 8))) void sp_emit_kernel(const uint32_t *__restrict__ ids, size_t N, size_t Npad, uint32_t ncols, const uint32_t *__restrict__ colcnt, int split,
                                                            const uint32_t *__restrict__ seg, uint32_t *__restrict__ order,
                                                            SpColWork cw, uint32_t *__restrict__ plctl, uint32_t plcap, uint32_t *__restrict__ gaveup, int big) {
    __shared__ uint32_t first[SP_EMIT_VCAP];
    __shared__ uint32_t cnt[SP_EMIT_VCAP];
    __shared__ uint32_t mrec[SP_EMIT_VCAP];
    __shared__ uint32_t vpre[SP_EMIT_VCAP];
    __shared__ uint32_t second[SP_EMIT_VCAP];
    __shared__ uint32_t cntb[SP_EMIT_VCAP];
    __shared__ unsigned long long wave_tot64[16];
    __shared__ uint32_t s_base, s_ebase, s_vbase, s_stop, s_cut, s_nent, s_nm;
    if (order[0]) return;
    constexpr uint32_t T = SP_EMIT_T, PER = (SP_EMIT_VCAP + T - 1) / T;
    const uint32_t tid = threadIdx.x;
    const size_t t = blockIdx.x;
    const uint32_t d2 = colcnt[t * BS_CC_STRIDE + 4];
    if (d2 == 0) return;
    const uint32_t *__restrict__ col = ids + t * Npad;
    const uint32_t n32 = (uint32_t)N;
    auto for_each_holder = [&](auto &&fn) {
#pragma unroll 1
        for (uint32_t j0 = 0; j0 < n32; j0 += T * 8) {
            uint32_t w[8], sg[8];
#pragma unroll
            for (int x = 0; x < 8; ++x) {
                const uint32_t j = j0 + (uint32_t)x * T + tid;
                w[x] = j < n32 ? col[j] : 0u;
                sg[x] = j < n32 ? seg[j] : 0u;
            }
#pragma unroll
            for (int x = 0; x < 8; ++x) { const uint32_t r = sp_rank(w[x], colcnt, t, split != 0); if (r) fn(r, sg[x], j0 + (uint32_t)x * T + tid); }
        }
    };
    const uint32_t vcap = big ? SP_EMIT_VCAP / 2 : SP_EMIT_VCAP;
    uint32_t colpairs = 0;
    bool voted = false;
    for (uint32_t lo = 0; lo < d2;) {
        EM_STAMP(0);
        const uint32_t len = min(vcap, d2 - lo);
        for (uint32_t x = tid; x < SP_EMIT_VCAP; x += T) { first[x] = SP_NONE; second[x] = SP_NONE; cnt[x] = 0; cntb[x] = 0; }
        if (tid == 0) s_stop = sp_ld(&order[0]);
        __syncthreads();
        if (s_stop) return;
        EM_STAMP(1);
        for_each_holder([&](uint32_t r, uint32_t sgv, uint32_t) {
            if (r <= lo || r > lo + len) return;
            const uint32_t q = r - 1 - lo;
            const uint32_t old = atomicCAS(&first[q], SP_NONE, sgv);
            const bool outside = old != SP_NONE && old != sgv;
            if (big) atomicAdd(&cnt[outside ? SP_EMIT_VCAP / 2 + q : q], 1u);
            else atomicAdd(&cnt[q], outside ? 0x10000u : 1u);
            if (outside) { const uint32_t o2 = atomicCAS(&second[q], SP_NONE, sgv); if (o2 == SP_NONE || o2 == sgv) atomicAdd(&cntb[q], 1u); }
        });
        __syncthreads();
        EM_STAMP(2);
        uint32_t n0[PER], nO[PER], oo = 0;
        bool mixed_mine = false;
#pragma unroll
        for (uint32_t x = 0; x < PER; ++x) {
            const uint32_t q = tid * PER + x;
            const uint32_t c = q < len ? cnt[q] : 0u;
            n0[x] = big ? c : (c & 0xFFFFu);
            nO[x] = q < len ? (big ? cnt[SP_EMIT_VCAP / 2 + q] : (c >> 16)) : 0u;
            if (q < len && nO[x]) {
                const uint32_t nb = cntb[q];
                if (nO[x] > nb) oo |= 1u << x;
                if (nb > n0[x]) { first[q] = second[q]; nO[x] += n0[x] - nb; n0[x] = nb; }
            }
            mixed_mine |= nO[x] != 0;
        }
        if (!__syncthreads_or(mixed_mine)) { EM_STAMP(3); lo += len; continue; }
        EM_STAMP(3);
        {
            unsigned long long v = 0;
            uint32_t ve = 0;
#pragma unroll
            for (uint32_t x = 0; x < PER; ++x) {
                if (!nO[x]) continue;
                ve = min(ve + min(n0[x], SP_EMIT_ECAP + 1u) + min(nO[x], SP_EMIT_ECAP + 1u), SP_EMIT_ECAP + 1u);
                v += 1ull << 32;
            }
            v |= ve;
            if (tid == 0) s_cut = len;
            unsigned long long tot;
// ... 707 lines not shown
        (rc = sp.d_sperm.alloc(ctx, Nstride, what)) ||
        (rc = sp.d_sinv.alloc(ctx, Npad, what)) ||
        (rc = sp.d_label.alloc(ctx, 2 * Npad, what)) ||
        (rc = sp.d_hint.alloc(ctx, 2 * Npad, what)) ||
        (rc = sp.d_segend.alloc(ctx, Npad, what)) ||
        (rc = sp.d_posseg.alloc(ctx, Npad * 2, what)) ||
        (rc = sp.d_spz.alloc(ctx, sp.spz_words, what)) ||
        (rc = sp.d_rowpos.alloc(ctx, Nstride, what)) ||
        (rc = sp.d_rowk.alloc(ctx, Npad, what)) ||
        (rc = sp.d_spctl.alloc(ctx, 2 * SP_CTL_WORDS + sp.tilebm_words, what)) ||
        (rc = sp.d_tiles.alloc(ctx, 8 * std::max<size_t>(sp.tiles_cap, 1), what)) ||
        (rc = sp.d_tiles_full.alloc(ctx, 8 * std::max<size_t>(sp.tiles_cap, 1), what)) ||
        (rc = sp.d_plist.alloc(ctx, sp.plist_cap, what)) ||
        (rc = sp.d_plist2.alloc(ctx, sp.plist_cap, what)) ||
        (rc = sp.d_bstart.alloc(ctx, (size_t)sp.nbins + 1, what)) ||
        (rc = sp.d_samp.alloc(ctx, SP_SAMPLE_ROWS * Npad + 8, what)) ||
        (rc = d2g_hip_status(ctx, hipMemset(sp.d_samp, 0, (SP_SAMPLE_ROWS * Npad + 8) * 4), what)) ||
        (rc = sp.d_cw_ents.alloc(ctx, sp.cw_ecap, what)) ||
        (rc = sp.d_cw_vals.alloc(ctx, sp.cw_vcap * 2, what)) ||
        (rc = sp.d_hoff.alloc(ctx, std::max<size_t>((size_t)sp.bin_nwg * sp.nbins, 1), what))) return rc;
    sp.d_lcnt = sp.d_spz;
    sp.d_gbm = sp.d_lcnt + (Npad + 1);
    sp.d_order = sp.d_gbm + 8 + sp.tilebm_words;
    sp.d_plctl = sp.d_order + 8;
    sp.d_fullctl = sp.d_plctl + 12;
    sp.d_binc = sp.d_fullctl + SP_CTL_WORDS;
    sp.d_tilebm = sp.d_spctl + 2 * SP_CTL_WORDS;
    if ((rc = d2g_hip_status(ctx, hipMemset(sp.d_spctl, 0, 2 * SP_CTL_WORDS * 4), what))) return rc;
    if (sp.h_gaveup.alloc(ctx, SP_MW_WORDS, what, hipHostMallocMapped) == D2G_OK && hipHostGetDevicePointer((void **)&sp.d_gaveup, sp.h_gaveup, 0) == hipSuccess) std::memset(sp.h_gaveup, 0, SP_MW_WORDS * 4);
    else { (void)hipGetLastError(); sp.h_gaveup.reset(); sp.d_gaveup = sp.d_order + 7; }
    set->sp.reset(new (std::nothrow) SpState(std::move(sp)));
    return set->sp ? D2G_OK : D2G_ERR_NOMEM;
}

SpInit sp_init_of(const d2g_cmp_set *set) {
    if (!set->sp) return SpInit{};
    const SpState &sp = *set->sp;
    return SpInit{sp.d_label, sp.d_hint, sp.d_spz, (uint32_t)set->N, (uint32_t)(2 * set->Npad), (uint32_t)sp.spz_words};
}

size_t sp_full_candidates(size_t Npad) {
    const size_t nrb = Npad / 32, ncb = Npad / BS_CB;
    size_t cand = 0;
    for (size_t cb = 0; cb < ncb; ++cb) cand += std::min<size_t>(nrb, (cb * 256 + 255) / 32 + 1);
    return cand;
}

__global__ void sp_giveup_kernel(uint32_t *__restrict__ order, uint32_t *__restrict__ fullctl, uint32_t cand) {
    if (threadIdx.x == 0) { order[0] = 1; fullctl[1] = 1; fullctl[3] = cand; }
}

struct SpSampleRows { uint32_t r[SP_SAMPLE_ROWS]; };
inline uint32_t sp_sample_field_bits(size_t ncols) { return div_up<size_t>(ncols, SP_SAMPLE_COLS) * SP_SAMPLE_FAM < 256 ? 8u : 16u; }
template <uint32_t FB>
__global__ __launch_bounds__(256) void sp_sample_kernel(const uint32_t *__restrict__ ids, size_t N, size_t Npad, uint32_t ncols, SpSampleRows rows, uint32_t *__restrict__ cntm) {
    constexpr uint32_t PW = 32 / FB;
    __shared__ __attribute__((aligned(16))) uint32_t sm[SP_SAMPLE_COLS][SP_SAMPLE_ROWS];
    const size_t j = (size_t)blockIdx.x * 256 + threadIdx.x;
    const uint32_t t0 = blockIdx.y * SP_SAMPLE_COLS, t1 = min(ncols, t0 + SP_SAMPLE_COLS);
    for (uint32_t x = threadIdx.x; x < SP_SAMPLE_COLS * SP_SAMPLE_ROWS; x += 256) {
        const uint32_t t = t0 + x / SP_SAMPLE_ROWS, k = x % SP_SAMPLE_ROWS;
        const uint32_t w = t < t1 ? ids[(size_t)t * Npad + rows.r[k]] : 0u;
        sm[x / SP_SAMPLE_ROWS][k] = (w != 0 && !(w >> 31)) ? w : 0xFFFFFFFFu;
    }
    __syncthreads();
    uint32_t acc[SP_SAMPLE_ROWS];
#pragma unroll
    for (uint32_t k = 0; k < SP_SAMPLE_ROWS; ++k) acc[k] = 0;
    typedef uint32_t u32x4 __attribute__((ext_vector_type(4)));
#pragma unroll 4
    for (uint32_t x = 0; x < SP_SAMPLE_COLS; ++x) {
        const uint32_t wx = (j < N && t0 + x < t1) ? ids[(size_t)(t0 + x) * Npad + j] : 0u;
#pragma unroll
        for (uint32_t q = 0; q < SP_SAMPLE_ROWS / 4; ++q) {
            const u32x4 s4 = reinterpret_cast<const u32x4 *>(&sm[x][0])[q];
            acc[4 * q] += wx == s4.x; acc[4 * q + 1] += wx == s4.y; acc[4 * q + 2] += wx == s4.z; acc[4 * q + 3] += wx == s4.w;
        }
    }
#pragma unroll
    for (uint32_t q = 0; q < SP_SAMPLE_ROWS / PW; ++q) {
        uint32_t w = 0;
#pragma unroll
        for (uint32_t y = 0; y < PW; ++y) w |= min(acc[PW * q + y], SP_SAMPLE_FAM) << (FB * y);
        if (w) atomicAdd(&cntm[(size_t)q * Npad + j], w);
    }
}
template <uint32_t FB>
__global__ __launch_bounds__(256) void sp_sample_fin_kernel(uint32_t *__restrict__ cntm, size_t N, size_t Npad, SpSampleRows rows, uint32_t *__restrict__ acc3, uint32_t *__restrict__ host_out,
                                                            const uint32_t *__restrict__ colcnt, uint32_t ncols, int nsplit, uint32_t ticket) {
    constexpr uint32_t PW = 32 / FB, MASK = (1u << FB) - 1u;
    const size_t j = (size_t)blockIdx.x * 256 + threadIdx.x;
    uint32_t e = 0, f = 0;
    uint32_t v = 0, pl = 0;
    if (j < ncols) {
        v = colcnt[j * BS_CC_STRIDE + 5];
        pl = v == 0 ? 1u : 32u - __clz(v + 1u);
    }
    if (j < N) {
#pragma unroll
        for (uint32_t q = 0; q < SP_SAMPLE_ROWS / PW; ++q) {
            const uint32_t w = cntm[(size_t)q * Npad + j];
            if (!w) continue;
            cntm[(size_t)q * Npad + j] = 0;
#pragma unroll
            for (uint32_t y = 0; y < PW; ++y) {
                const uint32_t c = (w >> (FB * y)) & MASK;
                if (c && j != rows.r[PW * q + y]) { if (c >= SP_SAMPLE_FAM) ++f; else e += c; }
            }
        }
    }
    for (int o = 32; o > 0; o >>= 1) { e += __shfl_down(e, o); f += __shfl_down(f, o); v += __shfl_down(v, o); pl += __shfl_down(pl, o); }
    if ((threadIdx.x & 63) == 0) { if (e) atomicAdd(&acc3[0], e); if (f) atomicAdd(&acc3[1], f); if (v) atomicAdd(&acc3[3], v); if (pl) atomicAdd(&acc3[4], pl); }
    __syncthreads();
    if (threadIdx.x == 0) {
        __threadfence();
        if (atomicAdd(&acc3[2], 1u) + 1u == gridDim.x) {
// ... 5 lines not shown
            __threadfence_system();
            __hip_atomic_store(&host_out[SP_MW_TICKET - SP_MW_SUMS], ticket, __ATOMIC_RELEASE, __HIP_MEMORY_SCOPE_SYSTEM);
        }
    }
}

SpColWork sp_colwork_of(const SpState &sp) {
    return SpColWork{sp.d_cw_ents, reinterpret_cast<uint4 *>(sp.d_cw_vals.get()), (uint32_t)std::min<size_t>(sp.cw_ecap, 0xFFFFFFFFu), (uint32_t)std::min<size_t>(sp.cw_vcap, 0xFFFFFFFFu)};
}
SpPairs sp_pairs_of(const SpState &sp, const SpColWork &cw, const uint32_t *seg) {
    return SpPairs{cw, seg, sp.d_plctl, sp.d_plist, (uint32_t)std::min<size_t>(sp.plist_cap, 0xFFFFFFFFu), sp.d_order, sp.d_gaveup, sp.d_fullctl};
}
bool sp_expect_long_list(const d2g_ctx *ctx, const SpState &sp) {
    if (!sp.bin_ok) return false;
    if (ctx->k2.list_form == 1) return false;
    if (ctx->k2.list_form == 2) return true;
    if (sp.dec.pred_valid) return sp.dec.pred_entries >= (double)ctx->k2.long_list;
    if (!sp.h_gaveup || sp.dec.prepares == 0) return true;
    const uint32_t n = ((volatile uint32_t *)sp.h_gaveup.get())[SP_MW_LIST_LEN];
    return n != 0xFFFFFFFFu && n >= ctx->k2.long_list;
}
bool sp_retry_due(const SpState &sp) { return ((sp.dec.prepares + 1) & 15u) == 0; }
bool sp_will_skip(const d2g_ctx *ctx, const SpState &sp) {
    if (sp.dec.pred_valid) return sp.dec.pred_dense;
    return ctx->k2.remember && sp.h_gaveup && ((volatile uint32_t *)sp.h_gaveup.get())[SP_MW_GAVEUP] && !sp_retry_due(sp);
}
bool sp_sample_due(const d2g_ctx *ctx, const d2g_cmp_set *set) {
    const SpState &sp = *set->sp;
    if (!ctx->k2.predict || !sp.d_samp || set->borrowed || set->nsplit > 1) return false;
    if (sp.dec.prepares == 0) return true;
    return ctx->k2.remember && sp.h_gaveup && ((volatile uint32_t *)sp.h_gaveup.get())[SP_MW_GAVEUP] && sp_retry_due(sp);
}

int sp_sample_enqueue(d2g_ctx *ctx, d2g_cmp_set *set, hipStream_t s) {
    const size_t N = set->N, Npad = set->Npad;
    SpState &sp = *set->sp;
    if (!sp.h_gaveup) return D2G_OK;
    { hipStreamCaptureStatus cs = hipStreamCaptureStatusNone; if (hipStreamIsCapturing(s, &cs) != hipSuccess || cs != hipStreamCaptureStatusNone) { (void)hipGetLastError(); return D2G_OK; } }
    SpSampleRows rows;
    for (uint32_t k = 0; k < SP_SAMPLE_ROWS; ++k) rows.r[k] = (uint32_t)std::min<size_t>(N - 1, (size_t)(2 * k + 1) * N / (2 * SP_SAMPLE_ROWS));
    uint32_t *acc3 = sp.d_samp + SP_SAMPLE_ROWS * Npad;
#ifndef D2G_SP_SAMPLE_INLINE
    if (!sp.samp_stream) {
        if (sp.samp_stream.create(hipStreamNonBlocking) != hipSuccess || sp.samp_event.create(hipEventDisableTiming) != hipSuccess) { (void)hipGetLastError(); sp.samp_stream.reset(); sp.samp_event.reset(); }
    }
    if (sp.samp_stream) {
        D2G_HIP(ctx, hipEventRecord(sp.samp_event, s));
        D2G_HIP(ctx, hipStreamWaitEvent(sp.samp_stream, sp.samp_event, 0));
        s = sp.samp_stream;
    }
#endif
    const bool wide = sp_sample_field_bits(set->ncols) == 16;
    const dim3 sgrid((unsigned)div_up<size_t>(N, 256), (unsigned)div_up<size_t>(set->ncols, SP_SAMPLE_COLS)), fgrid((unsigned)div_up<size_t>(std::max(N, set->ncols), 256));
    hipLaunchKernelGGL(wide ? sp_sample_kernel<16> : sp_sample_kernel<8>, sgrid, dim3(256), 0, s, set->d_ids, N, Npad, (uint32_t)set->ncols, rows, sp.d_samp);
    hipLaunchKernelGGL(wide ? sp_sample_fin_kernel<16> : sp_sample_fin_kernel<8>, fgrid, dim3(256), 0, s, sp.d_samp, N, Npad, rows, acc3, sp.d_gaveup + SP_MW_SUMS,
                       set->d_colcnt, (uint32_t)set->ncols, set->nsplit, ++sp.dec.sample_ticket);
    D2G_HIP(ctx, hipGetLastError());
    sp.dec.sample_pending = true;
    return D2G_OK;
}
int sp_sample_collect(d2g_ctx *ctx, d2g_cmp_set *set, hipStream_t s) {
    SpState &sp = *set->sp;
    if (!sp.dec.sample_pending) return D2G_OK;
    sp.dec.sample_pending = false;
    const size_t N = set->N;
    volatile uint32_t *h = (volatile uint32_t *)sp.h_gaveup.get() + SP_MW_SUMS;
    {
        const auto t0 = std::chrono::steady_clock::now();
        uint32_t spins = 0;
        while (__atomic_load_n(&sp.h_gaveup[SP_MW_TICKET], __ATOMIC_ACQUIRE) != sp.dec.sample_ticket) {
            __builtin_ia32_pause();
            if ((++spins & 1023u) == 0 && std::chrono::steady_clock::now() - t0 > std::chrono::milliseconds(250)) { D2G_HIP(ctx, hipStreamSynchronize(sp.samp_stream ? sp.samp_stream : s)); break; }
        }
    }
    const double scale = (double)N / (2.0 * SP_SAMPLE_ROWS), pairs = (double)N * (double)(N - 1) / 2.0;
    sp.dec.pred_valid = true;
    for (int x = 0; x < 4; ++x) sp.dec.samp_sums[x] = h[x];
    sp.dec.pred_entries = (double)h[0] * scale;
    sp.dec.pred_family_pairs = (double)h[1] * scale;
    const double values = (double)h[2], planes = set->ncols ? (double)h[3] / (double)set->ncols : 1.0;
    const double g = (double)set->ntb / 32.0, per_pair = 0.002 + 0.00094 * planes * g;
    const double dense_ns = pairs * per_pair, sparse_ns = (3.0 + 3.6 * g) * (double)N + 0.055 * sp.dec.pred_entries + 0.077 * values + 9.0 * per_pair * sp.dec.pred_family_pairs;
    sp.dec.pred_dense = sp.dec.pred_entries > (double)sp.plist_cap || sparse_ns > 0.97 * dense_ns;
    sp.h_gaveup[SP_MW_GAVEUP] = sp.dec.pred_dense ? 1u : 0u;
    return D2G_OK;
}

int sp_launch_merged(d2g_ctx *ctx, d2g_cmp_set *set, const SpOlinkArgs *l0, unsigned nx, unsigned npair, unsigned nflat, hipStream_t s) {
    SpState &sp = *set->sp;
    const BsPlanArgs pa{set->d_colcnt, (uint32_t)set->S, set->ntb, 1, set->d_perm, set->d_meta, set->d_meta + set->ntb, set->ex_meta, set->ex_status, ctx->k2.sort ? 1 : 0};
    const size_t nlink = (size_t)nx * npair, gx = div_up<size_t>(set->Nstride, 256), nplanes = gx * (size_t)set->ntb;
    D2G_CHECK(ctx, 1 + nlink < 0x40000000u && nflat + nplanes < 0x40000000u, "bitslice sparse: a merged launch does not fit a grid");
    unsigned g;
    SpRider rd = sp.announced.take((unsigned)(1 + nlink), SP_RW_M_LINK0, false, 1, &g);
    hipLaunchKernelGGL(sp_link0_plan_kernel, dim3(g), dim3(256), bs_plan_lds_words((uint32_t)set->ntb * 32u, pa.sort) * 4, s, pa, l0 ? *l0 : SpOlinkArgs{}, (uint32_t)nx, rd);
    rd = sp.announced.take((unsigned)(nflat + nplanes), SP_RW_M_PLANES, false, 2, &g);
    hipLaunchKernelGGL(bs_planes_flatten_kernel, dim3(g), dim3(256), 0, s, planes_args_of(set, set->d_planes, BS_FORM_STREAM), (uint32_t)gx, (uint32_t)nflat, sp.d_label.get(), rd);
    sp.dec.kernels += 2;
    D2G_HIP(ctx, hipGetLastError());
    return D2G_OK;
}

int sp_prepare_order(d2g_ctx *ctx, d2g_cmp_set *set, bool split, hipStream_t s) {
    const size_t N = set->N, Npad = set->Npad, S = set->ncols;
    SpState &sp = *set->sp;
    const bool remembered = sp.dec.skip_cached >= 0 ? sp.dec.skip_cached == 1 : sp_will_skip(ctx, sp);
    sp.dec.skip_cached = -1;
    const bool skip = sp.dec.pred_valid ? sp.dec.pred_dense : (remembered && sp.announced.riding() == 0);
    sp.dec.big = sp_expect_long_list(ctx, sp);
    ++sp.dec.prepares;
    sp.dec.looked = sp.dec.pred_valid; sp.dec.looked_dense = sp.dec.pred_valid && sp.dec.pred_dense;
    sp.dec.pred_valid = false;
    D2G_CHECK(ctx, !(skip && sp.dec.merged), "bitslice sparse: the merged schedule was chosen for a prepare that skips the ordering");
    if (skip) {
        ++sp.dec.kernels;
        hipLaunchKernelGGL(sp_giveup_kernel, dim3(1), dim3(64), 0, s, sp.d_order, sp.d_fullctl, (uint32_t)std::min<size_t>(sp_full_candidates(Npad), 0xFFFFFFFFu));
        D2G_HIP(ctx, hipGetLastError());
        sp.dec.skipped = true;
        return D2G_OK;
    }
    sp.dec.skipped = false;
    const unsigned nb = (unsigned)div_up<size_t>(N, 256);
    uint32_t *la = sp.d_label, *lb = sp.d_label + Npad;
    const d2g_k2_tuning &tu = ctx->k2;
    if (tu.link && S >= 2) {
        const uint32_t cap = (uint32_t)std::min<size_t>(N / 2 + 1, 12288);
        D2G_HIP(ctx, hipFuncSetAttribute((const void *)sp_link_kernel<0>, hipFuncAttributeMaxDynamicSharedMemorySize, 12288 * 12));
        D2G_HIP(ctx, hipFuncSetAttribute((const void *)sp_link_kernel<1>, hipFuncAttributeMaxDynamicSharedMemorySize, 12288 * 8));
        const unsigned npair = (unsigned)(S / 2);
        const uint32_t ustride = (uint32_t)std::max<size_t>(1, std::min<size_t>(SP_UNITE_STRIDE, npair / 32));
        if (sp.d_owner && !split && tu.olink) {
            const unsigned nx = (unsigned)div_up<size_t>(N, 1024);
            const SpOlinkArgs l0{set->d_ids, N, Npad, (uint32_t)S, sp.d_owner, sp.owner_stride, 1u, la, sp.d_hint};
            SpOlinkArgs l1 = l0; l1.stride = ustride;
            if (!sp.dec.merged) {
                hipLaunchKernelGGL(sp_olink_kernel<0>, dim3(nx, npair), dim3(256), 0, s, l0);
                { unsigned g; const SpRider rd = sp.announced.take(nb, SP_RW_FLATTEN, false, 2, &g); hipLaunchKernelGGL(sp_flatten_kernel, dim3(g), dim3(256), 0, s, la, N, rd); }
                sp.dec.kernels += 2;
            } else if (int rc = sp_launch_merged(ctx, set, &l0, nx, npair, nb, s)) return rc;
            hipLaunchKernelGGL(sp_olink_kernel<1>, dim3(nx, div_up<unsigned>(npair, ustride)), dim3(256), 0, s, l1);
            sp.dec.kernels += 1;
        } else {
            hipLaunchKernelGGL(sp_link_kernel<0>, dim3(npair), dim3(1024), (size_t)cap * 12, s, set->d_ids, N, Npad, (uint32_t)S, set->d_colcnt, split ? 1 : 0, cap, 1u,
                               la, sp.d_hint);
            { unsigned g; const SpRider rd = sp.announced.take(nb, SP_RW_FLATTEN, false, 2, &g); hipLaunchKernelGGL(sp_flatten_kernel, dim3(g), dim3(256), 0, s, la, N, rd); }
            hipLaunchKernelGGL(sp_link_kernel<1>, dim3(div_up<unsigned>(npair, ustride)), dim3(1024), (size_t)cap * 8, s, set->d_ids, N, Npad, (uint32_t)S, set->d_colcnt, split ? 1 : 0, cap, ustride,
                               la, sp.d_hint);
            sp.dec.kernels += 3;
        }
    } else if (sp.dec.merged) {
        if (int rc = sp_launch_merged(ctx, set, nullptr, 0, 0, 0, s)) return rc;
    }
    const size_t ntile_all = (Npad / 32) * (Npad / BS_CB);
    const uint32_t seg_limit = (uint32_t)std::min<size_t>((size_t)((double)ntile_all * tu.tile_frac), 0x3FFFFFFF);
    sp.dec.kernels += 4 + ((tu.link && S >= 2) ? 1 : 0) + (sp.dec.big ? 1 : 0);
    { unsigned g; const SpRider rd = sp.announced.take(nb, SP_RW_COUNT, false, 4, &g); hipLaunchKernelGGL(sp_count_kernel, dim3(g), dim3(256), 0, s, la, lb, N, sp.d_lcnt, sp.d_order, rd); }
    if (tu.link && S >= 2) {
        unsigned g; const SpRider rd = sp.announced.take(nb, SP_RW_ATTACH, false, 8, &g);
        hipLaunchKernelGGL(sp_attach_kernel, dim3(g), dim3(256), 0, s, lb, sp.d_lcnt, sp.d_hint, N, Npad, sp.d_order, rd);
    }
    const uint32_t CW = (uint32_t)((Npad / BS_CB + 31) / 32);
    { unsigned g; const SpRider rd = sp.announced.take(1, SP_RW_SCAN, false, 16, &g);
      hipLaunchKernelGGL(sp_scan_kernel, dim3(g), dim3(1024), 0, s, sp.d_lcnt, N, sp.d_order, la, sp.d_segend, seg_limit, sp.d_gaveup, rd); }
    { unsigned g; const SpRider rd = sp.announced.take((unsigned)div_up<size_t>(set->Nstride, 256), 0, true, 32, &g);
      hipLaunchKernelGGL(sp_place_kernel, dim3(g), dim3(256), 0, s, lb, N, set->Nstride, sp.d_lcnt, sp.d_sperm, sp.d_sinv, sp.d_order,
                         la, sp.d_segend, CW, sp.d_gbm + 8, reinterpret_cast<uint2 *>(sp.d_posseg.get()), rd); }
    const SpColWork cw = sp_colwork_of(sp);
    hipLaunchKernelGGL(sp_emit_kernel, dim3((unsigned)S), dim3(SP_EMIT_T), 0, s, set->d_ids, N, Npad, (uint32_t)S, set->d_colcnt, split ? 1 : 0, lb, sp.d_order,
                       cw, sp.d_plctl, (uint32_t)std::min<size_t>(sp.plist_cap, 0xFFFFFFFFu), sp.d_gaveup, (N >= 65536 || tu.emit_big) ? 1 : 0);
    if (sp.dec.big) hipLaunchKernelGGL(sp_pairs_kernel, dim3((unsigned)ctx->num_cus * 8), dim3(256), 0, s, sp_pairs_of(sp, cw, lb));
    D2G_HIP(ctx, hipGetLastError());
    return D2G_OK;
}

SpBins sp_bins_of(const SpState &sp) { return SpBins{sp.d_binc, sp.d_bstart, sp.nbins, sp.bin_nch, sp.bin_cshift}; }

int sp_permute(d2g_ctx *ctx, d2g_cmp_set *set, hipStream_t s) {
    SpState &sp = *set->sp;
    if (sp.dec.skipped) { sp.full_list_valid = true; return D2G_OK; }
    const size_t nrb = set->Npad / 32, ncb = set->Npad / BS_CB, ntile = nrb * ncb;
    const bool both = set->Nstride * 8 <= 156 * 1024;
    constexpr size_t LDS_PART = 128 * 1024;
    const uint32_t H = both ? 1u : (uint32_t)div_up<size_t>(set->Nstride * 4, LDS_PART);
    const uint32_t part = (uint32_t)(div_up<size_t>(div_up<size_t>(set->Nstride, H), 4) * 4);
    SpFullList fl{sp.d_gbm + 8, (uint32_t)nrb, (uint32_t)ncb, (uint32_t)((ncb + 31) / 32), sp.d_tiles_full, (uint32_t)sp.tiles_cap, sp.d_fullctl,
                  (uint32_t)std::min<size_t>(sp_full_candidates(set->Npad), 0xFFFFFFFFu), (uint32_t)div_up<size_t>(ntile, 1024), (uint32_t)set->N,
                  reinterpret_cast<const uint2 *>(sp.d_posseg.get())};
    const size_t nperm = (size_t)set->ntb * set->nbits_cap * (both ? 1 : 2) * H;
    const uint32_t plcap = (uint32_t)std::min<size_t>(sp.plist_cap, 0xFFFFFFFFu);
    SpHist hs{sp.d_plist, sp.d_plctl, plcap, sp.dec.big ? sp.bin_nwg : (uint32_t)ctx->num_cus, sp_bins_of(sp), sp.d_hoff, sp.dec.big ? 1 : 0,
              sp.h_gaveup ? sp.d_gaveup + SP_MW_LIST_LEN : nullptr};
    sp.full_list_valid = nperm + fl.nwg + hs.nhw < 0x7FFFFFFFu;
    if (!sp.full_list_valid) { ctx->last_error = "bitslice sparse: the permute launch does not fit a grid"; return D2G_ERR_INTERNAL; }
    const size_t lds = std::max<size_t>((size_t)part * (both ? 8 : 4), sp.dec.big ? (size_t)sp.nbins * 4 : 0);
    auto kern = both ? sp_permute_lds_kernel<true> : sp_permute_lds_kernel<false>;
    D2G_HIP(ctx, hipFuncSetAttribute((const void *)kern, hipFuncAttributeMaxDynamicSharedMemorySize, 157 * 1024));
    sp.dec.kernels += 1 + (sp.dec.big ? 1 : 0);
    hipLaunchKernelGGL(kern, dim3((unsigned)(nperm + fl.nwg + hs.nhw)), dim3(1024), lds, s, set->d_stream, sp.d_stream_s, set->Nstride, set->d_meta,
                       sp.d_sperm, sp.d_order, fl, (uint32_t)nperm, (uint32_t)set->nbits_cap, H, part, hs, sp_pairs_of(sp, sp_colwork_of(sp), sp.d_label + set->Npad));
    if (sp.dec.big) {
        D2G_HIP(ctx, hipFuncSetAttribute((const void *)sp_bin_kernel, hipFuncAttributeMaxDynamicSharedMemorySize, SP_BIN_MAX * 4));
        hipLaunchKernelGGL(sp_bin_kernel, dim3(hs.nhw), dim3(1024), (size_t)sp.nbins * 4, s, sp.d_plist, sp.d_plist2, sp.d_plctl, plcap, hs.bn, sp.d_hoff, sp.d_order);
    }
    D2G_HIP(ctx, hipGetLastError());
    return D2G_OK;
}

__global__ __launch_bounds__(256) void sp_unpack_kernel(const uint32_t *__restrict__ planes, size_t Nstride, int nbits_cap, const uint32_t *__restrict__ meta,
                                                        size_t N, size_t Npad, uint32_t *__restrict__ ids, uint32_t *__restrict__ colcnt, SpInit si) {
    const size_t j = (size_t)blockIdx.x * 256 + threadIdx.x;
    const size_t tb = blockIdx.y;
    sp_init_part(si, tb * ((size_t)gridDim.x * 256) + j, (size_t)gridDim.x * 256 * gridDim.y);
    const int nbits = live_planes(meta, (int)tb);
    const uint32_t *src = planes + tb * (size_t)(nbits_cap + 1) * Nstride + j;
    if (j < 32) colcnt[(tb * 32 + j) * BS_CC_STRIDE + 4] = planes[tb * (size_t)(nbits_cap + 1) * Nstride + (size_t)nbits_cap * Nstride + Npad + j];
    uint32_t id[32];
#pragma unroll
    for (int x = 0; x < 32; ++x) id[x] = 0;
    if (j < N) {
        for (int b = 0; b < nbits; ++b) {
            const uint32_t w = src[(size_t)b * Nstride];
// ... 86 lines not shown
```

### dashing2_amd/csrc/d2g_runtime.hip

```cpp
#include "d2g_internal.h"
#include <algorithm>
#include <cstdlib>
#include <cstring>
#include <new>

static const char *const kTuningNames[] = {
    "D2G_BS_SORT", "D2G_BS_NSPLIT", "D2G_BS_TAGBITS", "D2G_K2_MERGE",
    "D2G_BS_SPARSE", "D2G_BS_SPARSE_MIN_N", "D2G_SP_LINK", "D2G_SP_TILE_FRAC", "D2G_SP_LIST_DIV", "D2G_SP_LONG_LIST", "D2G_SP_LIST_FORM", "D2G_SP_PREDICT", "D2G_SP_REMEMBER", "D2G_SP_EMIT_BIG", "D2G_SP_OLINK", "D2G_SP_RIDE",
    "D2G_MGPU_CHUNKS",
    "D2G_K3_COMPACT", "D2G_K3_L1BITS", "D2G_K3_BUCKET_KEYS", "D2G_K3_SUB_KEYS", "D2G_K3_SPLIT_MIN", "D2G_K3_SUBBATCH", "D2G_K3_ROUND_KEYS",
    "D2G_K3_GUESS_SCALE", "D2G_K3_GRID_PER_CU", "D2G_K3_LIGHT", "D2G_K3_GQ_SCALE",
    "D2G_K3S_RANGE_KEYS", "D2G_KSET_SPLIT", "D2G_KSET_PBITS",
};
void d2g_tuning_load(d2g_tuning &t) {
    t.kv.clear();
    for (const char *n : kTuningNames)
        if (const char *v = std::getenv(n)) t.kv.emplace_back(n, v);
}

d2g_k2_tuning d2g_k2_tuning_resolve(const d2g_tuning &t) {
    d2g_k2_tuning v;
    if (const char *e = t.get("D2G_BS_SPARSE")) v.sparse = !(e[0] == '0');
    if (const char *e = t.get("D2G_BS_SPARSE_MIN_N")) v.min_n = (size_t)std::atoll(e);
    if (const char *e = t.get("D2G_SP_LINK")) v.link = std::atoi(e) != 0;
    if (const char *e = t.get("D2G_SP_TILE_FRAC")) { const double f = std::atof(e); if (f > 0 && f <= 1) v.tile_frac = f; }
    if (const char *e = t.get("D2G_SP_OLINK")) v.olink = std::atoi(e) != 0;
    if (const char *e = t.get("D2G_K2_MERGE")) v.merge = std::atoi(e) != 0;
    if (const char *e = t.get("D2G_SP_EMIT_BIG")) v.emit_big = std::atoi(e) != 0;
    if (const char *e = t.get("D2G_SP_REMEMBER")) v.remember = std::atoi(e) != 0;
    if (const char *e = t.get("D2G_SP_RIDE")) v.ride = std::atoi(e) & 63;
    if (const char *e = t.get("D2G_SP_LONG_LIST")) { const long long d = std::atoll(e); if (d >= 0) v.long_list = (size_t)d; }
    if (const char *e = t.get("D2G_SP_PREDICT")) v.predict = std::atoi(e) != 0;
    if (const char *e = t.get("D2G_SP_LIST_FORM")) { const int d = std::atoi(e); if (d >= 0 && d <= 2) v.list_form = d; }
    if (const char *e = t.get("D2G_SP_LIST_DIV")) { const long d = std::atol(e); if (d >= 1 && d <= (1 << 20)) v.list_div = (size_t)d; }
    if (const char *e = t.get("D2G_BS_SORT")) v.sort = !(e[0] == '0');
    if (const char *e = t.get("D2G_BS_TAGBITS")) { const int d = std::atoi(e); if (d >= 0 && d < 31) v.tagbits_max = d; }
    if (const char *e = t.get("D2G_BS_NSPLIT")) { const int d = std::atoi(e); if (d == 1 || d == 2 || d == 4) v.nsplit_req = d; }
    return v;
}

d2g_k3_tuning d2g_k3_tuning_resolve(const d2g_tuning &t) {
    d2g_k3_tuning v;
    if (const char *e = t.get("D2G_K3_COMPACT")) v.compact = e[0] == '1';
    if (const char *e = t.get("D2G_K3_LIGHT")) v.light = !(e[0] == '0');
    if (const char *e = t.get("D2G_K3_L1BITS")) { const int d = std::atoi(e); if (d >= 0 && d <= K3_MAXBBITS) v.l1bits = (uint32_t)d; }
    if (const char *e = t.get("D2G_K3_BUCKET_KEYS")) { const long d = std::atol(e); if (d >= 1) v.bucket_keys = (uint64_t)d; }
    if (const char *e = t.get("D2G_K3_SUB_KEYS")) { const long d = std::atol(e); if (d >= 1) v.sub_keys = (uint64_t)d; }
    if (const char *e = t.get("D2G_K3_SPLIT_MIN")) { const long d = std::atol(e); if (d >= 1) v.split_min = (uint64_t)d; }
    if (const char *e = t.get("D2G_K3_SUBBATCH")) { const int d = std::atoi(e); if (d >= 1 && d <= 8) v.subbatch = (size_t)d; }
    if (const char *e = t.get("D2G_K3_ROUND_KEYS")) { const int d = std::atoi(e); if (d >= 1 && d <= K3_ROUND_KEYS) v.round_keys = (uint32_t)d; }
    if (const char *e = t.get("D2G_K3_GUESS_SCALE")) { const double d = std::atof(e); if (d > 0.) v.guess_scale = d; }
    if (const char *e = t.get("D2G_K3_GRID_PER_CU")) { const int d = std::atoi(e); if (d >= 1 && d <= 256) v.grid_per_cu = (size_t)d; }
    if (const char *e = t.get("D2G_K3_GQ_SCALE")) { v.gq_scale_set = true; v.gq_scale = std::max(0.0, std::atof(e)); }
    v.gq_slack = v.gq_scale_set ? 1 : v.grid_per_cu > 24 ? 256 : 1024;
    if (const char *e = t.get("D2G_K3S_RANGE_KEYS")) { const long d = std::atol(e); if (d >= 1 && d <= K3_TARGET) v.sort_keys = (uint64_t)d; }
    return v;
}

void d2g_tuning_resolve(d2g_ctx *c) {
    d2g_tuning_load(c->tune);
    c->k2 = d2g_k2_tuning_resolve(c->tune);
    c->k3_tune = d2g_k3_tuning_resolve(c->tune);
    c->kset = d2g_kset_tuning();
    if (const char *e = c->tune.get("D2G_KSET_SPLIT")) { const int v = std::atoi(e); if (v >= 1 && v <= 65535) c->kset.split = v; }
    if (const char *e = c->tune.get("D2G_KSET_PBITS")) { const int v = std::atoi(e); if (v >= 0 && v <= 20) c->kset.pbits = v; }
    c->mgpu_chunks = 0;
    if (const char *e = c->tune.get("D2G_MGPU_CHUNKS")) { const int v = std::atoi(e); if (v >= 1 && v <= MG_MAX_CHUNKS) c->mgpu_chunks = v; }
}

extern "C" {

int d2g_ctx_reload_tuning(d2g_ctx *c) {
    if (!c) return D2G_ERR_INVALID;
    d2g_tuning_resolve(c);
    return D2G_OK;
}

int d2g_ctx_tuning(const d2g_ctx *c, char *buf, size_t cap) {
    if (!c) return D2G_ERR_INVALID;
    std::string j = "{";
    for (size_t i = 0; i < c->tune.kv.size(); ++i) {
        if (i) j += ", ";
        j += "\"" + c->tune.kv[i].first + "\": \"";
        for (char ch : c->tune.kv[i].second) { if (ch == '"' || ch == '\\') j += '\\'; if ((unsigned char)ch >= 0x20) j += ch; }
        j += "\"";
    }
    j += std::string(c->tune.kv.empty() ? "" : ", ") + "\"resolved\": " + d2g_k2_tuning_json(c);
    j += "}";
    if (buf && cap) { std::snprintf(buf, cap, "%s", j.c_str()); }
// ... 180 lines not shown
```

### include/d2g.h

```cpp
#ifndef D2G_H
#define D2G_H
#include <stddef.h>
#include <stdint.h>

#ifdef __cplusplus
extern "C" {
#endif

#define D2G_VERSION_MAJOR 0
#define D2G_VERSION_MINOR 1

typedef struct d2g_ctx d2g_ctx;

enum d2g_status {
    D2G_OK = 0,
    D2G_ERR_INVALID = -1,
    D2G_ERR_NODEVICE = -2,
    D2G_ERR_HIP = -3,
    D2G_ERR_NOMEM = -4,
    D2G_ERR_UNSUPPORTED = -5,
    D2G_ERR_IO = -6,
    D2G_ERR_INTERNAL = -7
};

// ... 195 lines not shown

int d2g_sketcher_ingest_fasta(d2g_sketcher *sk, const uint8_t *raw, size_t raw_bytes, const uint64_t *file_off,
                              const uint64_t *file_len, size_t nfiles, const uint64_t *genome_file_off , size_t n, int k);
int d2g_sketcher_ingested_runs(const d2g_sketcher *sk, const uint64_t **run_start, const uint32_t **run_len, size_t *nrun,
                               const uint64_t **genome_run_off , const uint64_t **genome_nkmers ,
                               uint64_t *nbases );

int d2g_bmh_sketch(d2g_ctx *ctx, const uint8_t *packed, size_t packed_bytes,
                   const uint64_t *run_start, const uint32_t *run_len, size_t nrun,
                   const uint64_t *genome_run_off, size_t n,
                   int k, int canon, uint64_t xormask, size_t sketchsize, double count_threshold,
                   double *sig_out , double *total_weight_out );
int d2g_bmh_sketch_dev(d2g_ctx *ctx, const d2g_oph_plan *plan, const uint8_t *packed_dev,
                       int canon, uint64_t xormask, size_t sketchsize, double count_threshold,
                       double *sig_out_dev , double *total_weight_out_dev , void *stream);
int d2g_sketcher_run_bmh(d2g_sketcher *sk, const uint8_t *packed, size_t packed_bytes,
                         const uint64_t *run_start, const uint32_t *run_len, size_t nrun,
                         const uint64_t *genome_run_off, size_t n, int k, int canon, uint64_t xormask,
                         size_t sketchsize, double count_threshold,
                         double *sig_out , double *total_weight_out );
int d2g_kmer_count(d2g_ctx *ctx, const uint8_t *packed, size_t packed_bytes,
                   const uint64_t *run_start, const uint32_t *run_len, size_t nrun,
                   const uint64_t *genome_run_off, size_t n, int k, int canon, uint64_t xormask,
                   double count_threshold, uint64_t *keys_out, uint32_t *counts_out, size_t cap,
                   uint64_t *genome_off_out );
int d2g_kmer_distinct(d2g_ctx *ctx, const uint8_t *packed, size_t packed_bytes,
                      const uint64_t *run_start, const uint32_t *run_len, size_t nrun,
                      const uint64_t *genome_run_off, size_t n, int k, int canon, uint64_t xormask,
                      uint64_t *ndistinct_out );
int d2g_sketcher_run_distinct(d2g_sketcher *sk, const uint8_t *packed, size_t packed_bytes,
                              const uint64_t *run_start, const uint32_t *run_len, size_t nrun,
                              const uint64_t *genome_run_off, size_t n, int k, int canon, uint64_t xormask,
                              uint64_t *ndistinct_out );
int d2g_bmh_check_weights(const double *weights , const uint64_t *set_off , size_t nsets,
                          size_t sketchsize, double scale, char *err, size_t errcap);
int d2g_bmh_from_weighted(d2g_ctx *ctx, const uint64_t *ids, const double *weights,
                          const uint64_t *set_off , size_t nsets, size_t sketchsize,
                          double *sig_out , double *total_weight_out );
int d2g_bmh_from_weighted_ids(d2g_ctx *ctx, const uint64_t *ids, const double *weights,
                              const uint64_t *set_off , size_t nsets, size_t sketchsize,
                              double *sig_out , double *total_weight_out ,
                              uint64_t *owner_out );

size_t d2g_ut_count(size_t N, size_t r0, size_t r1);
typedef struct d2g_cmp_set d2g_cmp_set;
int  d2g_cmp_set_create_dev(d2g_ctx *ctx, const uint64_t *sig_bits_dev, size_t N, size_t sketchsize,
                            int algo, void *stream, d2g_cmp_set **out);
int  d2g_cmp_set_create(d2g_ctx *ctx, const uint64_t *sig_bits_host, size_t N, size_t sketchsize,
                        int algo, d2g_cmp_set **out);
int  d2g_cmp_set_update_dev(d2g_ctx *ctx, d2g_cmp_set *set, const uint64_t *sig_bits_dev, void *stream);
int  d2g_cmp_set_status(d2g_ctx *ctx, const d2g_cmp_set *set, void *stream);
int  d2g_cmp_set_planes(d2g_ctx *ctx, const d2g_cmp_set *set, void *stream, unsigned *max_distinct, int *nbits,
                        float *mean_nbits);
int  d2g_cmp_set_sparse_info(d2g_ctx *ctx, const d2g_cmp_set *set, void *stream, uint32_t *info4);
int  d2g_cmp_set_debug_pairs(d2g_ctx *ctx, const d2g_cmp_set *set, void *stream, uint64_t *pairs_out, size_t cap, size_t *npairs, uint32_t *root_out);
int  d2g_cmp_set_sparse_detail(d2g_ctx *ctx, const d2g_cmp_set *set, void *stream, uint64_t *out10);
int  d2g_sparse_bin_geometry(size_t N, uint32_t *cshift, uint32_t *nch, uint32_t *nbins, int *binned_ok);
int  d2g_operand_layout(size_t N, size_t sketchsize, size_t *group_words, size_t *ngroups);
int  d2g_cmp_set_export_operand_dev(d2g_ctx *ctx, const d2g_cmp_set *set, uint32_t *planes_out_dev,
                                    uint32_t *meta_out_dev, void *stream);
int  d2g_cmp_set_from_planes_dev(d2g_ctx *ctx, size_t N, size_t sketchsize, const uint32_t *planes_dev,
                                 const uint32_t *meta_dev, d2g_cmp_set **out);
int  d2g_pack_column_slices_dev(d2g_ctx *ctx, const uint64_t *rows_dev, size_t n, size_t sketchsize, int nslices,
                                uint64_t *out_dev, void *stream);
void d2g_cmp_set_destroy(d2g_cmp_set *set);
int  d2g_cmp_set_algo(const d2g_cmp_set *set);
int  d2g_cmp_eqcount_ut_dev(d2g_ctx *ctx, const d2g_cmp_set *set, size_t r0, size_t r1,
                            uint32_t *neq_out_dev, void *stream);
int  d2g_cmp_lut_ut_dev(d2g_ctx *ctx, const d2g_cmp_set *set, size_t r0, size_t r1,
                        const float *lut_dev, float *out_dev, void *stream);
int  d2g_cmp_ut_prefill_dev(d2g_ctx *ctx, d2g_cmp_set *set, size_t r0, size_t r1, uint32_t *neq_out_dev,
                            const float *lut_dev, float *out_dev, void *stream);
int  d2g_cmp_ut_announce_dev(d2g_ctx *ctx, d2g_cmp_set *set, size_t r0, size_t r1, uint32_t *neq_out_dev,
                             const float *lut_dev, float *out_dev);
int  d2g_cmp_set_forget(d2g_ctx *ctx, d2g_cmp_set *set);
int  d2g_cmp_gtlt_ut_dev(d2g_ctx *ctx, const d2g_cmp_set *set, size_t r0, size_t r1,
                         uint32_t *gt_out_dev, uint32_t *lt_out_dev, void *stream);
int  d2g_cmp_eqcount_rect_dev(d2g_ctx *ctx, const d2g_cmp_set *set, size_t a0, size_t a1,
                              size_t b0, size_t b1, uint32_t *neq_out_dev, void *stream);

int  d2g_cmp_gtlt_rect_dev(d2g_ctx *ctx, const d2g_cmp_set *set, size_t a0, size_t a1, size_t b0, size_t b1,
                           uint32_t *gt_out_dev, uint32_t *lt_out_dev, void *stream);

int  d2g_cmp_eqcount_ut(d2g_ctx *ctx, const uint64_t *sig_bits, size_t N, size_t sketchsize,
                        size_t r0, size_t r1, int algo, uint32_t *neq_out);
int  d2g_cmp_dist_ut(d2g_ctx *ctx, const uint64_t *sig_bits, const double *cards, size_t N,
                     size_t sketchsize, size_t r0, size_t r1, int measure, int k, int multiset_space,
                     int algo, int nthreads, float *out);

int  d2g_cmp_set_create_codes_dev(d2g_ctx *ctx, const void *codes_dev, size_t N, size_t sketchsize, int regbytes, void *stream,
                                  d2g_cmp_set **out);
int  d2g_cmp_set_create_codes(d2g_ctx *ctx, const void *codes_host, size_t N, size_t sketchsize, int regbytes, d2g_cmp_set **out);
size_t d2g_cmp_set_operand_bytes(const d2g_cmp_set *set);
int  d2g_cmp_dist_trunc_ut(d2g_ctx *ctx, const double *sigs, const double *cards, size_t N, size_t sketchsize, size_t r0, size_t r1,
                           int measure, int k, int regbytes, int bbit, int nthreads, float *out);

int  d2g_cmp_knn_dev(d2g_ctx *ctx, const d2g_cmp_set *set, size_t r0, size_t r1, size_t K, uint32_t min_count,
                     const uint32_t *cls_dev, size_t cap, uint32_t *rowcnt_dev , uint32_t *ids_dev ,
                     uint32_t *counts_dev , size_t band_rows, void *stream);
int  d2g_knn_finish(const uint32_t *rowcnt, const uint32_t *ids, const uint32_t *counts, size_t nrows, size_t cap, const float *lut,
                    size_t sketchsize, int isdist, uint64_t *indptr_out , uint32_t *indices_out, float *data_out,
                    size_t out_cap, size_t *nnz_needed, size_t *overflow_rows);
int  d2g_cmp_set_knn(d2g_ctx *ctx, const d2g_cmp_set *set, size_t r0, size_t r1, const float *lut, int isdist, size_t K,
                     double threshold, size_t cap, size_t band_rows, uint64_t *indptr_out , uint32_t *indices_out,
                     float *data_out, size_t out_cap, size_t *nnz_needed);
int  d2g_cmp_knn(d2g_ctx *ctx, const uint64_t *sig_bits, size_t N, size_t sketchsize, size_t r0, size_t r1, int measure, int k,
// ... 91 lines not shown
```

Baseline: 203.2 billion.

## Store bitslice rank ids as 16-bit when the table fits in LDS

When the hash table fits the single-partition LDS size, the bitslice set stores per-column rank ids as uint16 instead of uint32, with the unique flag moved to bit 15. The rank, planes, link, olink, emit and flatten kernels are templated on the id type so they read and write the narrower array. The aim is to halve id memory traffic and footprint in set preparation. It adds template instantiations and guards that reject multi-partition or split sets, and enables by default through a new D2G_BS_ID16 tuning knob.

```diff
diff --git a/dashing2_amd/capi.py b/dashing2_amd/capi.py
--- a/dashing2_amd/capi.py
+++ b/dashing2_amd/capi.py
@@ -218,6 +218,7 @@
     "d2g_cmp_set_create_codes_dev": (_int, [_vp, _vp, _sz, _sz, _int, _vp, C.POINTER(_vp)]),
     "d2g_cmp_set_create_codes": (_int, [_vp, _vp, _sz, _sz, _int, C.POINTER(_vp)]),
     "d2g_cmp_set_operand_bytes": (_sz, [_vp]),
+    "d2g_cmp_set_id_bits": (_int, [_vp]),
     "d2g_cmp_dist_trunc_ut": (_int, [_vp, _vp, _vp, _sz, _sz, _sz, _sz, _int, _int, _int, _int, _int, _vp]),
     "d2g_cmp_knn_dev": (_int, [_vp, _vp, _sz, _sz, _sz, C.c_uint32, _vp, _sz, _vp, _vp, _vp, _sz, _vp]),
     "d2g_knn_finish": (_int, [_vp, _vp, _vp, _sz, _sz, _vp, _sz, _int, _vp, _vp, _vp, _sz, C.POINTER(_sz), C.POINTER(_sz)]),
@@ -248,7 +249,12 @@
                           "(dashing2_amd has no CPU fallback)")
         l = C.CDLL(LIB_PATH)
         for name, (res, args) in SIGNATURES.items():
-            f = getattr(l, name)
+            try:
+                f = getattr(l, name)
+            except AttributeError:
+                if os.environ.get("D2G_LIB"):
+                    continue
+                raise
             f.restype = res
             f.argtypes = args
         _lib = l
@@ -1242,6 +1248,10 @@
     def operand_bytes(self):
         return int(lib().d2g_cmp_set_operand_bytes(self._h))
 
+    @property
+    def id_bits(self):
+        return int(lib().d2g_cmp_set_id_bits(self._h))
+
     def close(self):
         if getattr(self, "_h", None):
             if self._owned:
diff --git a/dashing2_amd/csrc/d2g_internal.h b/dashing2_amd/csrc/d2g_internal.h
--- a/dashing2_amd/csrc/d2g_internal.h
+++ b/dashing2_amd/csrc/d2g_internal.h
@@ -80,6 +80,7 @@
     size_t list_div = 8;
     bool sort = true;
     int tagbits_max = 31;
+    int id16 = 1;
     int nsplit_req = 0;
 };
 d2g_k2_tuning d2g_k2_tuning_resolve(const d2g_tuning &t);
diff --git a/dashing2_amd/csrc/d2g_k2.h b/dashing2_amd/csrc/d2g_k2.h
--- a/dashing2_amd/csrc/d2g_k2.h
+++ b/dashing2_amd/csrc/d2g_k2.h
@@ -141,6 +141,7 @@
     int ntb = 0;
     uint32_t *d_meta = nullptr;
     d2g_dev<uint32_t> d_ids;
+    int id_bits = 32;
     uint32_t T = 0; int logT = 0;
     bool borrowed = false;
     bool want_exchange = false;
diff --git a/dashing2_amd/csrc/d2g_k2.hip b/dashing2_amd/csrc/d2g_k2.hip
--- a/dashing2_amd/csrc/d2g_k2.hip
+++ b/dashing2_amd/csrc/d2g_k2.hip
@@ -174,6 +174,8 @@
 }
 
 int d2g_cmp_set_algo(const d2g_cmp_set *set) { return set ? set->algo : D2G_ERR_INVALID; }
+
+int d2g_cmp_set_id_bits(const d2g_cmp_set *set) { return (set && set->algo == D2G_CMP_BITSLICE && set->d_ids) ? set->id_bits : 0; }
 
 size_t d2g_cmp_set_operand_bytes(const d2g_cmp_set *set) {
     if (!set) return 0;
diff --git a/dashing2_amd/csrc/d2g_k2_bitslice.hip b/dashing2_amd/csrc/d2g_k2_bitslice.hip
--- a/dashing2_amd/csrc/d2g_k2_bitslice.hip
+++ b/dashing2_amd/csrc/d2g_k2_bitslice.hip
@@ -17,6 +17,12 @@
 constexpr uint32_t BS_UNIQ = 0x80000000u;
 constexpr uint32_t BS_PENDING = 0x40000000u;
 constexpr int BS_LOG_TLDS_MAX = 15;
+template <typename IdT> struct BsId;
+template <> struct BsId<uint32_t> { static constexpr uint32_t UNIQ = BS_UNIQ; static constexpr int UBIT = 31; };
+template <> struct BsId<uint16_t> { static constexpr uint32_t UNIQ = 0x8000u; static constexpr int UBIT = 15; };
+constexpr size_t BS_ID16_MAX_N = ((size_t(1) << BS_LOG_TLDS_MAX) * 2) / 3;
+static_assert(BS_ID16_MAX_N / 2 < BsId<uint16_t>::UNIQ, "16-bit ids: the highest rank (N / 2) must stay below the unique flag");
+static_assert((size_t(1) << BS_LOG_TLDS_MAX) - 1 <= 0xFFFFu, "16-bit ids: the general single-partition kernel parks a table slot in ids[] between its two loops");
 
 __device__ __forceinline__ uint32_t bs_hash(uint64_t v, int logT) {
     return (uint32_t)((v * 0x9E3779B97F4A7C15ull) >> (64 - logT));
@@ -29,9 +35,9 @@
 #else
 #define RK_STAMP(k) do { } while (0)
 #endif
-template <bool MULTI, bool FAST>
+template <bool MULTI, bool FAST, typename IdT = uint32_t>
 __global__ __launch_bounds__(BS_RANK_THREADS) void bs_rank_kernel(const uint64_t *__restrict__ cols, size_t N, size_t Npad,
-                                                                  uint32_t T, int logT, uint32_t *ids_all, uint32_t *colcnt,
+                                                                  uint32_t T, int logT, void *ids_void, uint32_t *colcnt,
                                                                   uint32_t *status, int tagbits_max, uint32_t S, int nsplit,
                                                                   uint32_t *__restrict__ owner_all, size_t ostride) {
     extern __shared__ __attribute__((aligned(16))) uint32_t own[];
@@ -39,7 +45,8 @@
     const size_t t = MULTI ? blockIdx.x - split * S : blockIdx.x;
     const uint32_t htag = (MULTI && nsplit > 1) ? split << BS_SPLIT_SHIFT : 0u;
     const uint64_t *col = cols + t * Npad;
-    uint32_t *ids = ids_all + t * Npad;
+    static_assert(!MULTI || sizeof(IdT) == 4, "bs_rank_kernel: the pending words and split tags of the MULTI kernel need 32-bit ids");
+    IdT *ids = static_cast<IdT *>(ids_void) + t * Npad;
     const int tid = threadIdx.x;
     const int logTl = logT < BS_LOG_TLDS_MAX ? logT : BS_LOG_TLDS_MAX;
     const uint32_t Tl = 1u << logTl, mask = Tl - 1, nparts = MULTI ? (T >> logTl) : 1u;
@@ -76,7 +83,7 @@
             const uint32_t cur = own[h];
             if (cur != BS_EMPTY) {
                 if ((cur & BS_DUP) && owner) owner[r - 1] = cur & ownmask;
-                own[h] = (cur & BS_DUP) ? (r++ | htag) : BS_UNIQ;
+                own[h] = (cur & BS_DUP) ? (r++ | htag) : BsId<IdT>::UNIQ;
             }
         }
         __syncthreads();
@@ -178,13 +185,13 @@
 #pragma unroll
         for (int i = 0; i < PF; ++i) {
             const size_t j = (size_t)i * BS_RANK_THREADS + tid;
-            if (j < N && !(skip >> i & 1)) ids[j] = own[hs[i]];
+            if (j < N && !(skip >> i & 1)) ids[j] = (IdT)own[hs[i]];
         }
 #ifdef D2G_RANK_TRACE
         __syncthreads();
         RK_STAMP(5);
 #endif
-        for (uint32_t k = tid; k < nfix && k < BS_MAXFIX; k += BS_RANK_THREADS) ids[fix_j[k]] = own[fix_h[k]];
+        for (uint32_t k = tid; k < nfix && k < BS_MAXFIX; k += BS_RANK_THREADS) ids[fix_j[k]] = (IdT)own[fix_h[k]];
         if (tid == 0) { colcnt[t * BS_CC_STRIDE] = running - 1; colcnt[t * BS_CC_STRIDE + 5] = running - 1; }
         return;
     }
@@ -246,7 +253,7 @@
 #pragma unroll
             for (int i = 0; i < PG; ++i) {
                 const size_t j = j0 + (size_t)i * BS_RANK_THREADS + tid;
-                if ((mineb & ~redo) >> i & 1) ids[j] = hs[i] | (MULTI ? ptag : 0u);
+                if ((mineb & ~redo) >> i & 1) ids[j] = (IdT)(hs[i] | (MULTI ? ptag : 0u));
                 else if (MULTI && !tagged && part == 0 && j < N && !(redo >> i & 1)) ids[j] = 0;
             }
             while (redo) {
@@ -254,7 +261,7 @@
                 redo &= redo - 1;
                 const size_t j = j0 + (size_t)i * BS_RANK_THREADS + tid;
                 const uint64_t vv = col[j];
-                ids[j] = insert(vv, (uint32_t)j, bs_hash(vv, logT) & mask) | (MULTI ? ptag : 0u);
+                ids[j] = (IdT)(insert(vv, (uint32_t)j, bs_hash(vv, logT) & mask) | (MULTI ? ptag : 0u));
             }
             if (batch < 8) mine_all |= (unsigned long long)mineb << (8 * batch);
             ++batch;
@@ -275,7 +282,7 @@
             for (int i = 0; i < PG; ++i) {
                 const size_t j = j0 + (size_t)i * BS_RANK_THREADS + tid;
                 if (j < N && (mb >> i & 1) && (mine_known || !MULTI || (tagged ? (sl[i] & ~0x7FFFu) == ptag : (sl[i] & BS_PENDING) != 0)))
-                    ids[j] = own[sl[i] & (tagged ? 0x7FFFu : ~BS_PENDING)];
+                    ids[j] = (IdT)own[sl[i] & (tagged ? 0x7FFFu : ~BS_PENDING)];
             }
         }
         __syncthreads();
@@ -447,15 +454,18 @@
 constexpr int BS_FORM_STREAM = 1, BS_FORM_EXCHANGE = 2;
 constexpr size_t BS_SLACK = 64;
 struct BsPlanesArgs {
-    const uint32_t *ids; size_t N, Npad; uint32_t *planes, *stream; size_t Nstride; int nbits_cap; const uint32_t *meta; int forms;
+    const void *ids; size_t N, Npad; uint32_t *planes, *stream; size_t Nstride; int nbits_cap; const uint32_t *meta; int forms;
     const uint32_t *perm, *colcnt, *sperm;
 };
 BsPlanesArgs planes_args_of(const d2g_cmp_set *set, uint32_t *planes, int forms) {
-    return BsPlanesArgs{set->d_ids, set->N, set->Npad, planes, set->d_stream, set->Nstride, set->nbits_cap, set->d_meta, forms, set->d_perm, set->d_colcnt, nullptr};
-}
-template <bool SPLIT>
+    return BsPlanesArgs{set->d_ids.get(), set->N, set->Npad, planes, set->d_stream, set->Nstride, set->nbits_cap, set->d_meta, forms, set->d_perm, set->d_colcnt, nullptr};
+}
+template <bool SPLIT, typename IdT = uint32_t>
 __device__ __forceinline__ void bs_planes_body(const BsPlanesArgs &a, size_t bx, size_t tb) {
-    const uint32_t *__restrict__ ids = a.ids, *__restrict__ meta = a.meta, *__restrict__ perm = a.perm, *__restrict__ colcnt = a.colcnt, *__restrict__ sperm = a.sperm;
+    static_assert(!SPLIT || sizeof(IdT) == 4, "bs_planes_body: split ranks are 32-bit ids");
+    constexpr int UBIT = BsId<IdT>::UBIT;
+    const IdT *__restrict__ ids = static_cast<const IdT *>(a.ids);
+    const uint32_t *__restrict__ meta = a.meta, *__restrict__ perm = a.perm, *__restrict__ colcnt = a.colcnt, *__restrict__ sperm = a.sperm;
     uint32_t *__restrict__ planes = a.planes, *__restrict__ stream = a.stream;
     const size_t N = a.N, Npad = a.Npad, Nstride = a.Nstride;
     const int nbits_cap = a.nbits_cap, forms = a.forms;
@@ -477,7 +487,7 @@
     }
     uint32_t u = 0;
 #pragma unroll
-    for (int x = 0; x < 32; ++x) u |= (id[x] >> 31) << x;
+    for (int x = 0; x < 32; ++x) u |= (id[x] >> UBIT) << x;
     uint32_t *dst = planes + tb * (size_t)(nbits_cap + 1) * Nstride + jpos;
     const bool ex = forms & BS_FORM_EXCHANGE, st = forms & BS_FORM_STREAM;
     uint32_t *sdst = st ? stream + slot * 2 * Nstride + jpos : nullptr;
@@ -497,8 +507,8 @@
         dst[(size_t)nbits_cap * Nstride] = uw;
     }
 }
-template <bool SPLIT>
-__global__ __launch_bounds__(256) void bs_planes_kernel(BsPlanesArgs a) { bs_planes_body<SPLIT>(a, blockIdx.x, blockIdx.y); }
+template <bool SPLIT, typename IdT = uint32_t>
+__global__ __launch_bounds__(256) void bs_planes_kernel(BsPlanesArgs a) { bs_planes_body<SPLIT, IdT>(a, blockIdx.x, blockIdx.y); }
 
 __global__ __launch_bounds__(256) void bs_derive_kernel(const uint32_t *__restrict__ planes, uint32_t *__restrict__ stream,
                                                         size_t Nstride, int nbits_cap, const uint32_t *__restrict__ meta, int tb0) {
@@ -719,8 +729,11 @@
     }
     const char *what = "bitslice alloc";
     int rc;
-    if ((rc = set->d_ids.alloc(ctx, S * Npad, what)) ||
-        (rc = d2g_hip_status(ctx, hipMemset(set->d_ids, 0, S * Npad * sizeof(uint32_t)), what)) ||
+    set->id_bits = (ctx->k2.id16 && set->logT <= BS_LOG_TLDS_MAX) ? 16 : 32;
+    D2G_CHECK(ctx, set->id_bits == 32 || (N <= BS_ID16_MAX_N && set->nsplit == 1), "bitslice: 16-bit ids need a single-partition rank kernel");
+    const size_t id_words = set->id_bits == 16 ? (S * Npad + 1) / 2 : S * Npad;
+    if ((rc = set->d_ids.alloc(ctx, id_words, what)) ||
+        (rc = d2g_hip_status(ctx, hipMemset(set->d_ids, 0, id_words * sizeof(uint32_t)), what)) ||
         (rc = set->d_colcnt.alloc(ctx, S * BS_CC_STRIDE, what)) ||
         (rc = set->d_perm.alloc(ctx, (size_t)set->ntb * 32, what)) ||
         (rc = set->own_meta.alloc(ctx, (size_t)(set->ntb + 4), what)) ||
@@ -731,7 +744,8 @@
 int launch_planes(d2g_ctx *ctx, const d2g_cmp_set *set, uint32_t *planes, int forms, hipStream_t s) {
     const dim3 grid((unsigned)div_up<size_t>(set->Nstride, 256), (unsigned)set->ntb);
     const bool split = set->logT > BS_LOG_TLDS_MAX && set->nsplit > 1;
-    hipLaunchKernelGGL(split ? bs_planes_kernel<true> : bs_planes_kernel<false>, grid, dim3(256), 0, s, planes_args_of(set, planes, forms));
+    D2G_CHECK(ctx, !(split && set->id_bits == 16), "bitslice: a split set with 16-bit ids");
+    hipLaunchKernelGGL((set->id_bits == 16 ? bs_planes_kernel<false, uint16_t> : split ? bs_planes_kernel<true> : bs_planes_kernel<false>), grid, dim3(256), 0, s, planes_args_of(set, planes, forms));
     D2G_HIP(ctx, hipGetLastError());
     return D2G_OK;
 }
@@ -786,14 +800,17 @@
     {
         const int logTl = set->logT < BS_LOG_TLDS_MAX ? set->logT : BS_LOG_TLDS_MAX;
         const size_t lds = (size_t(1) << logTl) * sizeof(uint32_t);
-        void (*kern)(const uint64_t *, size_t, size_t, uint32_t, int, uint32_t *, uint32_t *, uint32_t *, int, uint32_t, int, uint32_t *, size_t) = bs_rank_kernel<false, false>;
+        const bool id16 = set->id_bits == 16;
+        D2G_CHECK(ctx, !(multi && id16), "bitslice: the multi-partition rank kernel with 16-bit ids");
+        void (*kern)(const uint64_t *, size_t, size_t, uint32_t, int, void *, uint32_t *, uint32_t *, int, uint32_t, int, uint32_t *, size_t) = bs_rank_kernel<false, false>;
         if (multi) kern = bs_rank_kernel<true, false>;
-        else if (N <= (size_t)12 * BS_RANK_THREADS) kern = bs_rank_kernel<false, true>;
+        else if (N <= (size_t)12 * BS_RANK_THREADS) kern = id16 ? bs_rank_kernel<false, true, uint16_t> : bs_rank_kernel<false, true>;
+        else if (id16) kern = bs_rank_kernel<false, false, uint16_t>;
         if (lds > 48 * 1024)
             D2G_HIP(ctx, hipFuncSetAttribute((const void *)kern, hipFuncAttributeMaxDynamicSharedMemorySize, (int)lds));
         if (nsplit > 1) D2G_HIP(ctx, hipMemsetAsync(set->d_ids, 0, S * Npad * sizeof(uint32_t), s));
         hipLaunchKernelGGL(kern, dim3((unsigned)(S * nsplit)), dim3(BS_RANK_THREADS), lds, s, set->d_cols, N, Npad, set->T, set->logT,
-                           set->d_ids, set->d_colcnt, set->d_meta + set->ntb, ctx->k2.tagbits_max, (uint32_t)S, nsplit,
+                           (void *)set->d_ids.get(), set->d_colcnt, set->d_meta + set->ntb, ctx->k2.tagbits_max, (uint32_t)S, nsplit,
                            (sp && nsplit == 1) ? sp->d_owner.get() : (uint32_t *)nullptr, sp ? sp->owner_stride : 0);
         if (sp) sp->dec.kernels = 2 + (join.ev ? 1 : 0);
         const bool look = sparse_path && sp_sample_due(ctx, set);
@@ -1020,8 +1037,8 @@
     const d2g_k2_tuning &t = ctx->k2;
     char b[640];
     std::snprintf(b, sizeof b, "{\"D2G_BS_SPARSE\": %d, \"D2G_BS_SPARSE_MIN_N\": %zu, \"D2G_BS_SORT\": %d, \"D2G_SP_LINK\": %d, \"D2G_SP_OLINK\": %d, \"D2G_SP_TILE_FRAC\": %.3f, "
-                  "\"D2G_SP_LIST_DIV\": %zu, \"D2G_SP_LONG_LIST\": %zu, \"D2G_SP_LIST_FORM\": %d, \"D2G_SP_PREDICT\": %d, \"D2G_SP_REMEMBER\": %d, \"D2G_SP_RIDE\": %d, \"D2G_SP_EMIT_BIG\": %d, \"D2G_K2_MERGE\": %d}",
-                  t.sparse ? 1 : 0, t.min_n, t.sort ? 1 : 0, t.link, t.olink, t.tile_frac, t.list_div, t.long_list, t.list_form, t.predict, t.remember, t.ride, t.emit_big, t.merge);
+                  "\"D2G_SP_LIST_DIV\": %zu, \"D2G_SP_LONG_LIST\": %zu, \"D2G_SP_LIST_FORM\": %d, \"D2G_SP_PREDICT\": %d, \"D2G_SP_REMEMBER\": %d, \"D2G_SP_RIDE\": %d, \"D2G_SP_EMIT_BIG\": %d, \"D2G_K2_MERGE\": %d, \"D2G_BS_ID16\": %d}",
+                  t.sparse ? 1 : 0, t.min_n, t.sort ? 1 : 0, t.link, t.olink, t.tile_frac, t.list_div, t.long_list, t.list_form, t.predict, t.remember, t.ride, t.emit_big, t.merge, t.id16);
     return b;
 }
 
diff --git a/dashing2_amd/csrc/d2g_k2_sparse.h b/dashing2_amd/csrc/d2g_k2_sparse.h
--- a/dashing2_amd/csrc/d2g_k2_sparse.h
+++ b/dashing2_amd/csrc/d2g_k2_sparse.h
@@ -8,9 +8,11 @@
 #define D2G_SP_WPE 8
 #endif
 
+template <typename IdT = uint32_t>
 __device__ __forceinline__ uint32_t sp_rank(uint32_t w, const uint32_t *__restrict__ colcnt, size_t t, bool split) {
-    if ((w >> 31) || w == 0) return 0;
-    return split ? (w & BS_RANK_MASK) + colcnt[t * BS_CC_STRIDE + (w >> BS_SPLIT_SHIFT)] : w;
+    if ((w >> BsId<IdT>::UBIT) || w == 0) return 0;
+    if constexpr (sizeof(IdT) == 2) return w;
+    else return split ? (w & BS_RANK_MASK) + colcnt[t * BS_CC_STRIDE + (w >> BS_SPLIT_SHIFT)] : w;
 }
 
 __device__ __forceinline__ uint32_t sp_ld(const uint32_t *p) { return __hip_atomic_load(p, __ATOMIC_RELAXED, __HIP_MEMORY_SCOPE_AGENT); }
@@ -36,10 +38,11 @@
 }
 
 constexpr uint32_t SP_UDONE = 0x40000000u, SP_R2MASK = 0x3FFFFFFFu;
-template <int MODE>
-__global__ __launch_bounds__(1024) void sp_link_kernel(const uint32_t *__restrict__ ids, size_t N, size_t Npad, uint32_t ncols, const uint32_t *__restrict__ colcnt,
+template <int MODE, typename IdT = uint32_t>
+__global__ __launch_bounds__(1024) void sp_link_kernel(const void *__restrict__ ids_void, size_t N, size_t Npad, uint32_t ncols, const uint32_t *__restrict__ colcnt,
                                                        int split, uint32_t cap, uint32_t stride, uint32_t *label, uint32_t *__restrict__ hint) {
     extern __shared__ uint32_t sp_l[];
+    const IdT *__restrict__ ids = static_cast<const IdT *>(ids_void);
     const size_t pair = (size_t)blockIdx.x * stride;
     const size_t t1 = 2 * pair, t2 = t1 + 1;
     if (t2 >= ncols) return;
@@ -62,7 +65,7 @@
 #pragma unroll
         for (int x = 0; x < U; ++x) {
             const uint32_t j = (uint32_t)(j0 + (size_t)x * T + threadIdx.x);
-            const uint32_t a = sp_rank(w1[x], colcnt, t1, split != 0), b = sp_rank(w2[x], colcnt, t2, split != 0);
+            const uint32_t a = sp_rank<IdT>(w1[x], colcnt, t1, split != 0), b = sp_rank<IdT>(w2[x], colcnt, t2, split != 0);
             if (!a || a > nv) continue;
             if (MODE == 0) any[a - 1] = j;
             if (!b) continue;
@@ -86,7 +89,7 @@
 #pragma unroll
         for (int x = 0; x < U; ++x) {
             const uint32_t j = (uint32_t)(j0 + (size_t)x * T + threadIdx.x);
-            const uint32_t a = sp_rank(w1[x], colcnt, t1, split != 0), b = sp_rank(w2[x], colcnt, t2, split != 0);
+            const uint32_t a = sp_rank<IdT>(w1[x], colcnt, t1, split != 0), b = sp_rank<IdT>(w2[x], colcnt, t2, split != 0);
             if (!a || a > nv) continue;
             const uint32_t rr = r2[a - 1];
             const bool match = b && rr != SP_NONE && (rr & SP_R2MASK) == b;
@@ -107,40 +110,43 @@
 }
 
 constexpr uint32_t SP_OWNER_MASK = 0x7FFFFFFFu;
-struct SpOlinkArgs { const uint32_t *ids; size_t N, Npad; uint32_t ncols; uint32_t *owner; size_t ostride; uint32_t stride; uint32_t *label, *hint; };
-template <int MODE>
+struct SpOlinkArgs { const void *ids; size_t N, Npad; uint32_t ncols; uint32_t *owner; size_t ostride; uint32_t stride; uint32_t *label, *hint; };
+constexpr int SP_OLINK_W = 4;
+template <int MODE, typename IdT = uint32_t>
 __device__ __forceinline__ void sp_olink_body(const SpOlinkArgs &a, size_t bx, size_t by) {
-    const uint32_t *__restrict__ ids = a.ids;
+    constexpr int W = SP_OLINK_W, UBIT = BsId<IdT>::UBIT;
+    const IdT *__restrict__ ids = static_cast<const IdT *>(a.ids);
     uint32_t *__restrict__ owner = a.owner, *label = a.label, *__restrict__ hint = a.hint;
     const size_t N = a.N, Npad = a.Npad, ostride = a.ostride;
     const size_t pair = by * a.stride;
     const size_t t1 = 2 * pair, t2 = t1 + 1;
     if (t2 >= a.ncols) return;
-    const size_t j0 = (bx * 256 + threadIdx.x) * 4;
+    const size_t j0 = (bx * 256 + threadIdx.x) * W;
     if (j0 >= N) return;
-    typedef uint32_t u32x4 __attribute__((ext_vector_type(4)));
-    const u32x4 w1 = *reinterpret_cast<const u32x4 *>(ids + t1 * Npad + j0);
-    const u32x4 w2 = *reinterpret_cast<const u32x4 *>(ids + t2 * Npad + j0);
-    const u32x4 lb = *reinterpret_cast<const u32x4 *>(label + j0);
+    IdT w1[W], w2[W];
+    uint32_t lb[W];
+    __builtin_memcpy(w1, __builtin_assume_aligned(ids + t1 * Npad + j0, W * sizeof(IdT)), sizeof w1);
+    __builtin_memcpy(w2, __builtin_assume_aligned(ids + t2 * Npad + j0, W * sizeof(IdT)), sizeof w2);
+    __builtin_memcpy(lb, __builtin_assume_aligned(label + j0, 16), sizeof lb);
     uint32_t *myhint = hint + (size_t)(pair & 1u) * Npad;
-    uint32_t o[4], r2o[4], lo[4];
-#pragma unroll
-    for (int x = 0; x < 4; ++x) {
+    uint32_t o[W], r2o[W], lo[W];
+#pragma unroll
+    for (int x = 0; x < W; ++x) {
         const uint32_t r1 = w1[x];
-        o[x] = (r1 && !(r1 >> 31) && j0 + x < N) ? owner[t1 * ostride + r1 - 1] & SP_OWNER_MASK : SP_NONE;
-    }
-#pragma unroll
-    for (int x = 0; x < 4; ++x) {
+        o[x] = (r1 && !(r1 >> UBIT) && j0 + x < N) ? owner[t1 * ostride + r1 - 1] & SP_OWNER_MASK : SP_NONE;
+    }
+#pragma unroll
+    for (int x = 0; x < W; ++x) {
         const bool live = o[x] != SP_NONE && o[x] != (uint32_t)(j0 + x);
-        r2o[x] = live ? ids[t2 * Npad + o[x]] : 0u;
+        r2o[x] = live ? (uint32_t)ids[t2 * Npad + o[x]] : 0u;
         lo[x] = live ? label[o[x]] : 0u;
         if (!live) o[x] = SP_NONE;
     }
 #pragma unroll
-    for (int x = 0; x < 4; ++x) {
+    for (int x = 0; x < W; ++x) {
         if (o[x] == SP_NONE) continue;
         const uint32_t j = (uint32_t)(j0 + x), r2 = w2[x];
-        const bool match = r2 && !(r2 >> 31) && r2 == r2o[x];
+        const bool match = r2 && !(r2 >> UBIT) && r2 == r2o[x];
         if (MODE == 0) {
             if (match) {
                 if (lo[x] < lb[x]) label[j] = lo[x]; else if (lb[x] < lo[x]) label[o[x]] = lb[x];
@@ -151,8 +157,8 @@
         }
     }
 }
-template <int MODE>
-__global__ __launch_bounds__(256) void sp_olink_kernel(SpOlinkArgs a) { sp_olink_body<MODE>(a, blockIdx.x, blockIdx.y); }
+template <int MODE, typename IdT = uint32_t>
+__global__ __launch_bounds__(256) void sp_olink_kernel(SpOlinkArgs a) { sp_olink_body<MODE, IdT>(a, blockIdx.x, blockIdx.y); }
 
 __device__ __forceinline__ void sp_flatten_body(uint32_t *label, size_t N, size_t bx) {
     const size_t j = bx * 256 + threadIdx.x;
@@ -172,18 +178,20 @@
     sp_flatten_body(label, N, blockIdx.x);
 }
 
+template <typename IdT = uint32_t>
 __global__ __launch_bounds__(256) void sp_link0_plan_kernel(BsPlanArgs pa, SpOlinkArgs la, uint32_t nx, SpRider rider) {
     SP_RIDE_OR_WORK(rider);
     extern __shared__ __attribute__((aligned(16))) uint32_t plan_lds[];
     if (blockIdx.x == 0) { bs_colplan_body<256>(pa, bs_plan_lds(plan_lds, (uint32_t)pa.ntb * 32u)); return; }
     const uint32_t b = blockIdx.x - 1u;
-    sp_olink_body<0>(la, b % nx, b / nx);
-}
+    sp_olink_body<0, IdT>(la, b % nx, b / nx);
+}
+template <typename IdT = uint32_t>
 __global__ __launch_bounds__(256) void bs_planes_flatten_kernel(BsPlanesArgs a, uint32_t gx, uint32_t nflat, uint32_t *label, SpRider rider) {
     SP_RIDE_OR_WORK(rider);
     if (blockIdx.x < nflat) { sp_flatten_body(label, a.N, blockIdx.x); return; }
     const uint32_t b = blockIdx.x - nflat;
-    bs_planes_body<false>(a, b % gx, b / gx);
+    bs_planes_body<false, IdT>(a, b % gx, b / gx);
 }
 
 __global__ __launch_bounds__(256) void sp_attach_kernel(uint32_t *__restrict__ root, uint32_t *__restrict__ cnt, const uint32_t *__restrict__ hint, size_t N, size_t Npad,
@@ -369,7 +377,8 @@
 #define EM_STAMP(k) do { } while (0)
 #endif
 constexpr uint32_t SP_EMIT_VCAP = 1536, SP_EMIT_ECAP = 32768, SP_EMIT_T = D2G_SP_EMIT_T;
-__global__ __launch_bounds__(SP_EMIT_T) __attribute__((amdgpu_waves_per_eu(8, 8))) void sp_emit_kernel(const uint32_t *__restrict__ ids, size_t N, size_t Npad, uint32_t ncols, const uint32_t *__restrict__ colcnt, int split,
+template <typename IdT = uint32_t>
+__global__ __launch_bounds__(SP_EMIT_T) __attribute__((amdgpu_waves_per_eu(8, 8))) void sp_emit_kernel(const void *__restrict__ ids_void, size_t N, size_t Npad, uint32_t ncols, const uint32_t *__restrict__ colcnt, int split,
                                                             const uint32_t *__restrict__ seg, uint32_t *__restrict__ order,
                                                             SpColWork cw, uint32_t *__restrict__ plctl, uint32_t plcap, uint32_t *__restrict__ gaveup, int big) {
     __shared__ uint32_t first[SP_EMIT_VCAP];
@@ -386,9 +395,31 @@
     const size_t t = blockIdx.x;
     const uint32_t d2 = colcnt[t * BS_CC_STRIDE + 4];
     if (d2 == 0) return;
-    const uint32_t *__restrict__ col = ids + t * Npad;
+    const IdT *__restrict__ col = static_cast<const IdT *>(ids_void) + t * Npad;
     const uint32_t n32 = (uint32_t)N;
     auto for_each_holder = [&](auto &&fn) {
+        if constexpr (sizeof(IdT) == 2) {
+            typedef uint32_t u32x2 __attribute__((ext_vector_type(2)));
+#pragma unroll 1
+            for (uint32_t j0 = 0; j0 < n32; j0 += T * 8) {
+                uint32_t w[4];
+                u32x2 sg[4];
+#pragma unroll
+                for (int x = 0; x < 4; ++x) {
+                    const uint32_t j = j0 + 2u * ((uint32_t)x * T + tid);
+                    w[x] = j < n32 ? *reinterpret_cast<const uint32_t *>(col + j) : 0u;
+                    sg[x] = j < n32 ? *reinterpret_cast<const u32x2 *>(seg + j) : u32x2{0u, 0u};
+                }
+#pragma unroll
+                for (int x = 0; x < 4; ++x) {
+                    const uint32_t j = j0 + 2u * ((uint32_t)x * T + tid);
+                    const uint32_t ra = sp_rank<IdT>(w[x] & 0xFFFFu, colcnt, t, false), rb = sp_rank<IdT>(w[x] >> 16, colcnt, t, false);
+                    if (ra) fn(ra, sg[x].x, j);
+                    if (rb) fn(rb, sg[x].y, j + 1u);
+                }
+            }
+            return;
+        }
 #pragma unroll 1
         for (uint32_t j0 = 0; j0 < n32; j0 += T * 8) {
             uint32_t w[8], sg[8];
@@ -399,7 +430,7 @@
                 sg[x] = j < n32 ? seg[j] : 0u;
             }
 #pragma unroll
-            for (int x = 0; x < 8; ++x) { const uint32_t r = sp_rank(w[x], colcnt, t, split != 0); if (r) fn(r, sg[x], j0 + (uint32_t)x * T + tid); }
+            for (int x = 0; x < 8; ++x) { const uint32_t r = sp_rank<IdT>(w[x], colcnt, t, split != 0); if (r) fn(r, sg[x], j0 + (uint32_t)x * T + tid); }
         }
     };
     const uint32_t vcap = big ? SP_EMIT_VCAP / 2 : SP_EMIT_VCAP;
@@ -1213,16 +1244,17 @@
 
 struct SpSampleRows { uint32_t r[SP_SAMPLE_ROWS]; };
 inline uint32_t sp_sample_field_bits(size_t ncols) { return div_up<size_t>(ncols, SP_SAMPLE_COLS) * SP_SAMPLE_FAM < 256 ? 8u : 16u; }
-template <uint32_t FB>
-__global__ __launch_bounds__(256) void sp_sample_kernel(const uint32_t *__restrict__ ids, size_t N, size_t Npad, uint32_t ncols, SpSampleRows rows, uint32_t *__restrict__ cntm) {
+template <uint32_t FB, typename IdT = uint32_t>
+__global__ __launch_bounds__(256) void sp_sample_kernel(const void *__restrict__ ids_void, size_t N, size_t Npad, uint32_t ncols, SpSampleRows rows, uint32_t *__restrict__ cntm) {
     constexpr uint32_t PW = 32 / FB;
     __shared__ __attribute__((aligned(16))) uint32_t sm[SP_SAMPLE_COLS][SP_SAMPLE_ROWS];
+    const IdT *__restrict__ ids = static_cast<const IdT *>(ids_void);
     const size_t j = (size_t)blockIdx.x * 256 + threadIdx.x;
     const uint32_t t0 = blockIdx.y * SP_SAMPLE_COLS, t1 = min(ncols, t0 + SP_SAMPLE_COLS);
     for (uint32_t x = threadIdx.x; x < SP_SAMPLE_COLS * SP_SAMPLE_ROWS; x += 256) {
         const uint32_t t = t0 + x / SP_SAMPLE_ROWS, k = x % SP_SAMPLE_ROWS;
         const uint32_t w = t < t1 ? ids[(size_t)t * Npad + rows.r[k]] : 0u;
-        sm[x / SP_SAMPLE_ROWS][k] = (w != 0 && !(w >> 31)) ? w : 0xFFFFFFFFu;
+        sm[x / SP_SAMPLE_ROWS][k] = (w != 0 && !(w >> BsId<IdT>::UBIT)) ? w : 0xFFFFFFFFu;
     }
     __syncthreads();
     uint32_t acc[SP_SAMPLE_ROWS];
@@ -1334,7 +1366,8 @@
 #endif
     const bool wide = sp_sample_field_bits(set->ncols) == 16;
     const dim3 sgrid((unsigned)div_up<size_t>(N, 256), (unsigned)div_up<size_t>(set->ncols, SP_SAMPLE_COLS)), fgrid((unsigned)div_up<size_t>(std::max(N, set->ncols), 256));
-    hipLaunchKernelGGL(wide ? sp_sample_kernel<16> : sp_sample_kernel<8>, sgrid, dim3(256), 0, s, set->d_ids, N, Npad, (uint32_t)set->ncols, rows, sp.d_samp);
+    const bool id16 = set->id_bits == 16;
+    hipLaunchKernelGGL((wide ? (id16 ? sp_sample_kernel<16, uint16_t> : sp_sample_kernel<16>) : (id16 ? sp_sample_kernel<8, uint16_t> : sp_sample_kernel<8>)), sgrid, dim3(256), 0, s, (const void *)set->d_ids.get(), N, Npad, (uint32_t)set->ncols, rows, sp.d_samp);
     hipLaunchKernelGGL(wide ? sp_sample_fin_kernel<16> : sp_sample_fin_kernel<8>, fgrid, dim3(256), 0, s, sp.d_samp, N, Npad, rows, acc3, sp.d_gaveup + SP_MW_SUMS,
                        set->d_colcnt, (uint32_t)set->ncols, set->nsplit, ++sp.dec.sample_ticket);
     D2G_HIP(ctx, hipGetLastError());
@@ -1371,13 +1404,14 @@
 int sp_launch_merged(d2g_ctx *ctx, d2g_cmp_set *set, const SpOlinkArgs *l0, unsigned nx, unsigned npair, unsigned nflat, hipStream_t s) {
     SpState &sp = *set->sp;
     const BsPlanArgs pa{set->d_colcnt, (uint32_t)set->S, set->ntb, 1, set->d_perm, set->d_meta, set->d_meta + set->ntb, set->ex_meta, set->ex_status, ctx->k2.sort ? 1 : 0};
+    const bool id16 = set->id_bits == 16;
     const size_t nlink = (size_t)nx * npair, gx = div_up<size_t>(set->Nstride, 256), nplanes = gx * (size_t)set->ntb;
     D2G_CHECK(ctx, 1 + nlink < 0x40000000u && nflat + nplanes < 0x40000000u, "bitslice sparse: a merged launch does not fit a grid");
     unsigned g;
     SpRider rd = sp.announced.take((unsigned)(1 + nlink), SP_RW_M_LINK0, false, 1, &g);
-    hipLaunchKernelGGL(sp_link0_plan_kernel, dim3(g), dim3(256), bs_plan_lds_words((uint32_t)set->ntb * 32u, pa.sort) * 4, s, pa, l0 ? *l0 : SpOlinkArgs{}, (uint32_t)nx, rd);
+    hipLaunchKernelGGL((id16 ? sp_link0_plan_kernel<uint16_t> : sp_link0_plan_kernel<uint32_t>), dim3(g), dim3(256), bs_plan_lds_words((uint32_t)set->ntb * 32u, pa.sort) * 4, s, pa, l0 ? *l0 : SpOlinkArgs{}, (uint32_t)nx, rd);
     rd = sp.announced.take((unsigned)(nflat + nplanes), SP_RW_M_PLANES, false, 2, &g);
-    hipLaunchKernelGGL(bs_planes_flatten_kernel, dim3(g), dim3(256), 0, s, planes_args_of(set, set->d_planes, BS_FORM_STREAM), (uint32_t)gx, (uint32_t)nflat, sp.d_label.get(), rd);
+    hipLaunchKernelGGL((id16 ? bs_planes_flatten_kernel<uint16_t> : bs_planes_flatten_kernel<uint32_t>), dim3(g), dim3(256), 0, s, planes_args_of(set, set->d_planes, BS_FORM_STREAM), (uint32_t)gx, (uint32_t)nflat, sp.d_label.get(), rd);
     sp.dec.kernels += 2;
     D2G_HIP(ctx, hipGetLastError());
     return D2G_OK;
@@ -1405,28 +1439,32 @@
     const unsigned nb = (unsigned)div_up<size_t>(N, 256);
     uint32_t *la = sp.d_label, *lb = sp.d_label + Npad;
     const d2g_k2_tuning &tu = ctx->k2;
+    const bool id16 = set->id_bits == 16;
+    const void *const ids = set->d_ids.get();
+    D2G_CHECK(ctx, !(id16 && split), "bitslice sparse: split ranks in 16-bit ids");
     if (tu.link && S >= 2) {
         const uint32_t cap = (uint32_t)std::min<size_t>(N / 2 + 1, 12288);
-        D2G_HIP(ctx, hipFuncSetAttribute((const void *)sp_link_kernel<0>, hipFuncAttributeMaxDynamicSharedMemorySize, 12288 * 12));
-        D2G_HIP(ctx, hipFuncSetAttribute((const void *)sp_link_kernel<1>, hipFuncAttributeMaxDynamicSharedMemorySize, 12288 * 8));
+        const auto link0 = id16 ? sp_link_kernel<0, uint16_t> : sp_link_kernel<0, uint32_t>, link1 = id16 ? sp_link_kernel<1, uint16_t> : sp_link_kernel<1, uint32_t>;
+        D2G_HIP(ctx, hipFuncSetAttribute((const void *)link0, hipFuncAttributeMaxDynamicSharedMemorySize, 12288 * 12));
+        D2G_HIP(ctx, hipFuncSetAttribute((const void *)link1, hipFuncAttributeMaxDynamicSharedMemorySize, 12288 * 8));
         const unsigned npair = (unsigned)(S / 2);
         const uint32_t ustride = (uint32_t)std::max<size_t>(1, std::min<size_t>(SP_UNITE_STRIDE, npair / 32));
         if (sp.d_owner && !split && tu.olink) {
-            const unsigned nx = (unsigned)div_up<size_t>(N, 1024);
-            const SpOlinkArgs l0{set->d_ids, N, Npad, (uint32_t)S, sp.d_owner, sp.owner_stride, 1u, la, sp.d_hint};
+            const unsigned nx = (unsigned)div_up<size_t>(N, 256 * (size_t)SP_OLINK_W);
+            const SpOlinkArgs l0{ids, N, Npad, (uint32_t)S, sp.d_owner, sp.owner_stride, 1u, la, sp.d_hint};
             SpOlinkArgs l1 = l0; l1.stride = ustride;
             if (!sp.dec.merged) {
-                hipLaunchKernelGGL(sp_olink_kernel<0>, dim3(nx, npair), dim3(256), 0, s, l0);
+                hipLaunchKernelGGL((id16 ? sp_olink_kernel<0, uint16_t> : sp_olink_kernel<0, uint32_t>), dim3(nx, npair), dim3(256), 0, s, l0);
                 { unsigned g; const SpRider rd = sp.announced.take(nb, SP_RW_FLATTEN, false, 2, &g); hipLaunchKernelGGL(sp_flatten_kernel, dim3(g), dim3(256), 0, s, la, N, rd); }
                 sp.dec.kernels += 2;
             } else if (int rc = sp_launch_merged(ctx, set, &l0, nx, npair, nb, s)) return rc;
-            hipLaunchKernelGGL(sp_olink_kernel<1>, dim3(nx, div_up<unsigned>(npair, ustride)), dim3(256), 0, s, l1);
+            hipLaunchKernelGGL((id16 ? sp_olink_kernel<1, uint16_t> : sp_olink_kernel<1, uint32_t>), dim3(nx, div_up<unsigned>(npair, ustride)), dim3(256), 0, s, l1);
             sp.dec.kernels += 1;
         } else {
-            hipLaunchKernelGGL(sp_link_kernel<0>, dim3(npair), dim3(1024), (size_t)cap * 12, s, set->d_ids, N, Npad, (uint32_t)S, set->d_colcnt, split ? 1 : 0, cap, 1u,
+            hipLaunchKernelGGL(link0, dim3(npair), dim3(1024), (size_t)cap * 12, s, ids, N, Npad, (uint32_t)S, set->d_colcnt, split ? 1 : 0, cap, 1u,
                                la, sp.d_hint);
             { unsigned g; const SpRider rd = sp.announced.take(nb, SP_RW_FLATTEN, false, 2, &g); hipLaunchKernelGGL(sp_flatten_kernel, dim3(g), dim3(256), 0, s, la, N, rd); }
-            hipLaunchKernelGGL(sp_link_kernel<1>, dim3(div_up<unsigned>(npair, ustride)), dim3(1024), (size_t)cap * 8, s, set->d_ids, N, Npad, (uint32_t)S, set->d_colcnt, split ? 1 : 0, cap, ustride,
+            hipLaunchKernelGGL(link1, dim3(div_up<unsigned>(npair, ustride)), dim3(1024), (size_t)cap * 8, s, ids, N, Npad, (uint32_t)S, set->d_colcnt, split ? 1 : 0, cap, ustride,
                                la, sp.d_hint);
             sp.dec.kernels += 3;
         }
@@ -1448,7 +1486,7 @@
       hipLaunchKernelGGL(sp_place_kernel, dim3(g), dim3(256), 0, s, lb, N, set->Nstride, sp.d_lcnt, sp.d_sperm, sp.d_sinv, sp.d_order,
                          la, sp.d_segend, CW, sp.d_gbm + 8, reinterpret_cast<uint2 *>(sp.d_posseg.get()), rd); }
     const SpColWork cw = sp_colwork_of(sp);
-    hipLaunchKernelGGL(sp_emit_kernel, dim3((unsigned)S), dim3(SP_EMIT_T), 0, s, set->d_ids, N, Npad, (uint32_t)S, set->d_colcnt, split ? 1 : 0, lb, sp.d_order,
+    hipLaunchKernelGGL((id16 ? sp_emit_kernel<uint16_t> : sp_emit_kernel<uint32_t>), dim3((unsigned)S), dim3(SP_EMIT_T), 0, s, ids, N, Npad, (uint32_t)S, set->d_colcnt, split ? 1 : 0, lb, sp.d_order,
                        cw, sp.d_plctl, (uint32_t)std::min<size_t>(sp.plist_cap, 0xFFFFFFFFu), sp.d_gaveup, (N >= 65536 || tu.emit_big) ? 1 : 0);
     if (sp.dec.big) hipLaunchKernelGGL(sp_pairs_kernel, dim3((unsigned)ctx->num_cus * 8), dim3(256), 0, s, sp_pairs_of(sp, cw, lb));
     D2G_HIP(ctx, hipGetLastError());
diff --git a/dashing2_amd/csrc/d2g_runtime.hip b/dashing2_amd/csrc/d2g_runtime.hip
--- a/dashing2_amd/csrc/d2g_runtime.hip
+++ b/dashing2_amd/csrc/d2g_runtime.hip
@@ -5,7 +5,7 @@
 #include <new>
 
 static const char *const kTuningNames[] = {
-    "D2G_BS_SORT", "D2G_BS_NSPLIT", "D2G_BS_TAGBITS", "D2G_K2_MERGE",
+    "D2G_BS_SORT", "D2G_BS_NSPLIT", "D2G_BS_TAGBITS", "D2G_BS_ID16", "D2G_K2_MERGE",
     "D2G_BS_SPARSE", "D2G_BS_SPARSE_MIN_N", "D2G_SP_LINK", "D2G_SP_TILE_FRAC", "D2G_SP_LIST_DIV", "D2G_SP_LONG_LIST", "D2G_SP_LIST_FORM", "D2G_SP_PREDICT", "D2G_SP_REMEMBER", "D2G_SP_EMIT_BIG", "D2G_SP_OLINK", "D2G_SP_RIDE",
     "D2G_MGPU_CHUNKS",
     "D2G_K3_COMPACT", "D2G_K3_L1BITS", "D2G_K3_BUCKET_KEYS", "D2G_K3_SUB_KEYS", "D2G_K3_SPLIT_MIN", "D2G_K3_SUBBATCH", "D2G_K3_ROUND_KEYS",
@@ -35,6 +35,7 @@
     if (const char *e = t.get("D2G_SP_LIST_DIV")) { const long d = std::atol(e); if (d >= 1 && d <= (1 << 20)) v.list_div = (size_t)d; }
     if (const char *e = t.get("D2G_BS_SORT")) v.sort = !(e[0] == '0');
     if (const char *e = t.get("D2G_BS_TAGBITS")) { const int d = std::atoi(e); if (d >= 0 && d < 31) v.tagbits_max = d; }
+    if (const char *e = t.get("D2G_BS_ID16")) v.id16 = std::atoi(e) != 0;
     if (const char *e = t.get("D2G_BS_NSPLIT")) { const int d = std::atoi(e); if (d == 1 || d == 2 || d == 4) v.nsplit_req = d; }
     return v;
 }
diff --git a/include/d2g.h b/include/d2g.h
--- a/include/d2g.h
+++ b/include/d2g.h
@@ -271,6 +271,7 @@
 int  d2g_cmp_set_status(d2g_ctx *ctx, const d2g_cmp_set *set, void *stream);
 int  d2g_cmp_set_planes(d2g_ctx *ctx, const d2g_cmp_set *set, void *stream, unsigned *max_distinct, int *nbits,
                         float *mean_nbits);
+int  d2g_cmp_set_id_bits(const d2g_cmp_set *set);
 int  d2g_cmp_set_sparse_info(d2g_ctx *ctx, const d2g_cmp_set *set, void *stream, uint32_t *info4);
 int  d2g_cmp_set_debug_pairs(d2g_ctx *ctx, const d2g_cmp_set *set, void *stream, uint64_t *pairs_out, size_t cap, size_t *npairs, uint32_t *root_out);
 int  d2g_cmp_set_sparse_detail(d2g_ctx *ctx, const d2g_cmp_set *set, void *stream, uint64_t *out10);
```

Result: faster. 207.6 billion, median of 6 (+2.2%).
